# Erikx3/gym_dockauv

Hardware: AMD Instinct MI355X
Metric: env-steps/sec (batched docking3d) (higher is better)
Workload: dtype f32

## Files before the change

gym_dockauv_amd/csrc/dockauv_capi.hip:

```cpp
#include <algorithm>
#include <cmath>
#include <cstdarg>
#include <cstdio>
#include <cstring>

#include "dockauv_capi.h"

using namespace dockauv;

namespace dockauv {

thread_local std::string g_create_error;

int fail(dockauv_handle h, int code, const char* fmt, ...) {
    char buf[512];
    va_list ap;
    va_start(ap, fmt);
    vsnprintf(buf, sizeof buf, fmt, ap);
    va_end(ap);
    if (h) h->err = buf; else g_create_error = buf;
    return code;
}

int check_status(dockauv_handle h) {
    if (!h->status_host) return 0;
    const unsigned int v = *h->status_host;
    if (v != 0)
        return fail(h, DOCKAUV_E_KERNEL, "step kernel status 0x%x: a tail role timed out waiting for its group's integrating wave; "
                    "results since are invalid, destroy the handle", v);
    return 0;
}

int sync_last(dockauv_handle h) {
    if (h->last_stream) HIP_TRY(h, hipStreamSynchronize(h->last_stream)); else HIP_TRY(h, hipDeviceSynchronize());
    return 0;
}

}

namespace {

struct FieldDesc {
    void* base;
    int rows;
    int kind;
};

int dalloc(dockauv_handle h, void** p, size_t bytes) {
    if (bytes == 0) bytes = 256;
    hipError_t e = hipMalloc(p, bytes);
    if (e != hipSuccess) return fail(h, DOCKAUV_E_HIP, "hipMalloc(%zu) failed: %s", bytes, hipGetErrorString(e));
    e = hipMemset(*p, 0, bytes);
    if (e != hipSuccess) return fail(h, DOCKAUV_E_HIP, "hipMemset failed: %s", hipGetErrorString(e));
    h->allocs.push_back(*p);
    return 0;
}

template <typename T>
void fill_vehicle(VehicleP<T>& d, const dockauv_vehicle& v) {
    d.m = (T)v.m;
    d.gWB = (T)(v.W - v.BY);
    d.gx = (T)(v.r_G[0] * v.W - v.r_B[0] * v.BY);
    d.gy = (T)(v.r_G[1] * v.W - v.r_B[1] * v.BY);
    d.gz = (T)(v.r_G[2] * v.W - v.r_B[2] * v.BY);
    for (int i = 0; i < 3; ++i) d.rg[i] = (T)v.r_G[i];
    for (int i = 0; i < 9; ++i) d.Ib[i] = (T)v.I_b[i];
    for (int i = 0; i < 6; ++i) {
        d.ma[i] = (T)v.ma_diag[i];
        d.dl[i] = (T)v.d_lin[i];
        d.dq[i] = (T)v.d_quad[i];
    }
    for (int i = 0; i < 36; ++i) d.Minv[i] = (T)v.M_inv[i];
    for (int i = 0; i < 6 * kMaxU; ++i) d.B[i] = (T)v.B[i];
    for (int i = 0; i < kMaxU; ++i) {
        d.ulo[i] = (T)v.u_lo[i];
        d.uhalf[i] = (T)(v.u_hi[i] - v.u_lo[i]);
    }
    for (int i = 0; i < L_COUNT; ++i) d.lauv[i] = (T)v.lauv[i];
    {
        const double m = v.m, zg = v.r_G[2];
        const double* a = v.ma_diag;
        const double Ix = v.I_b[0], Iy = v.I_b[4], Iz = v.I_b[8];
        const double kc[10] = {m + a[0], m + a[1], m + a[2], m * zg,
                               Iy - Iz + a[4] - a[5], a[1] - a[2],
                               Iz - Ix + a[5] - a[3], a[2] - a[0],
                               Ix - Iy + a[3] - a[4], a[0] - a[1]};
        for (int i = 0; i < 10; ++i) d.kc[i] = (T)kc[i];
    }
    d.n_u = v.n_u;
}

template <typename T>
void fill_env(EnvP<T>& e, const dockauv_env_s& h) {
    const dockauv_config& c = h.cfg;
    e.n_envs = c.n_envs;
    e.max_timesteps = c.max_timesteps;
    e.reward_set = c.reward_set;
    e.reset_mode = c.reset_mode;
    e.scenario = c.scenario;
    e.n_v = c.n_v;
    e.n_h = c.n_h;
    e.blk = c.blocksize_reduce;
    e.n_vr = (c.n_v + c.blocksize_reduce - 1) / c.blocksize_reduce;
    e.n_hr = (c.n_h + c.blocksize_reduce - 1) / c.blocksize_reduce;
    e.n_rays = h.n_rays;
    e.n_red = h.n_red;
    e.n_obs = h.n_obs;
    e.max_cap = c.max_capsules;
    e.max_sph = c.max_spheres;
    e.n_u_max = h.n_u_max;
    e.bf16_wpr = (h.n_obs + 1) / 2 + 2;
    e.bf16_magic = (unsigned)((0x100000000ull / (unsigned)e.bf16_wpr) + 1ull);
    e.seed = c.seed;
    e.h = (T)c.t_step_size;
    e.lp_alpha = (T)(c.t_step_size / (c.t_step_size + c.lowpass_T1));
    e.mu = (T)c.current_mu;
    e.dmax = (T)c.max_dist_from_goal;
    e.dtol = (T)c.dist_goal_reached_tol;
    e.max_att = (T)c.max_attitude;
    e.safety = (T)c.safety_radius;
    for (int i = 0; i < 6; ++i) {
        e.vel_max[i] = (T)c.vel_max[i];
        e.inv_vel[i] = (T)(1.0 / c.vel_max[i]);
    }
    const double eps = 0.001;
    e.inv_dmax = (T)(1.0 / c.max_dist_from_goal);
    e.inv_log_tol = (T)(1.0 / std::log(c.dist_goal_reached_tol / c.max_dist_from_goal));
    e.inv_log_tol_eps = (T)(1.0 / std::log(std::max(c.dist_goal_reached_tol, eps) / c.max_dist_from_goal));
    e.inv_max_att = (T)(1.0 / c.max_attitude);
    e.inv_ray_max = (T)(1.0 / c.radar_max_dist);
    e.w_d = (T)c.w_d;
    e.w_dth = (T)c.w_delta_theta;
    e.w_dpsi = (T)c.w_delta_psi;
    e.w_phi = (T)c.w_phi;
    e.w_th = (T)c.w_theta;
    e.w_thdot = (T)c.w_Thetadot;
    e.w_oa = (T)c.w_oa;
    for (int i = 0; i < 5; ++i) e.w_done[i] = (T)c.w_done[i];
    for (int i = 0; i < kMaxU; ++i) e.w_act[i] = (T)c.action_reward_factors[i];
    e.ray_max = (T)c.radar_max_dist;
    e.alpha_max = (T)c.radar_alpha_max;
    e.beta_max = (T)c.radar_beta_max;
    e.ray_pad_log2 = ceil_log2(h.n_rays);
    e.ray_pad = 1 << e.ray_pad_log2;
    e.device_noise = c.device_noise ? 1 : 0;
    e.fan_cos = (T)h.fan_cos;
    e.fan_sin = (T)h.fan_sin;
    e.sum_beta = (T)h.sum_beta;
}

bool is_symmetric_vehicle(const dockauv_vehicle& v) {
    if (v.r_G[0] != 0.0 || v.r_G[1] != 0.0 || v.r_B[0] != 0.0 || v.r_B[1] != 0.0) return false;
    for (int i = 0; i < 3; ++i)
        for (int j = 0; j < 3; ++j)
            if (i != j && v.I_b[i * 3 + j] != 0.0) return false;
    for (int i = 0; i < 6; ++i)
        for (int j = 0; j < 6; ++j) {
            const bool allowed = (i == j) || (i == 0 && j == 4) || (i == 4 && j == 0) || (i == 1 && j == 3) || (i == 3 && j == 1);
            if (!allowed && std::fabs(v.M_inv[i * 6 + j]) > 1e-14 * std::fabs(v.M_inv[i * 6 + i])) return false;
        }
    return true;
}

bool b_is_diagonal(const dockauv_vehicle& v) {
    if (v.n_u != 6) return false;
    for (int i = 0; i < 6; ++i)
        for (int j = 0; j < kMaxU; ++j)
            if (i != j && v.B[i * kMaxU + j] != 0.0) return false;
    return true;
}

int field_info(dockauv_handle h, int field, FieldDesc* fd, int* width) {
    const dockauv_config& c = h->cfg;
    switch (field) {
        case DOCKAUV_F_STATE: *fd = {h->B.state, 12, 0}; *width = 12; return 0;
        case DOCKAUV_F_U: *fd = {h->B.u, kMaxU, 0}; *width = kMaxU; return 0;
        case DOCKAUV_F_GOAL: *fd = {h->B.goal, 4, 0}; *width = 4; return 0;
        case DOCKAUV_F_CURRENT: *fd = {h->B.cur, 8, 0}; *width = 5; return 0;
        case DOCKAUV_F_TSTEPS: *fd = {h->B.t_steps, 1, 1}; *width = 1; return 0;
        case DOCKAUV_F_CAPSULES: *fd = {h->B.caps, c.max_capsules * 7, 0}; *width = c.max_capsules * 7; return 0;
        case DOCKAUV_F_SPHERES: *fd = {h->B.sph, c.max_spheres * 4, 0}; *width = c.max_spheres * 4; return 0;
        case DOCKAUV_F_VEHICLE_ID: *fd = {h->B.veh_id, 1, 2}; *width = 1; return 0;
        case DOCKAUV_F_CUM_REWARD: *fd = {h->B.cum_reward, 1, 0}; *width = 1; return 0;
        case DOCKAUV_F_EPISODE: *fd = {h->B.episode, 1, 1}; *width = 1; return 0;
        case DOCKAUV_F_CURRENT_SIGMA: *fd = {h->B.cur_sigma, 1, 0}; *width = 1; return 0;
        case DOCKAUV_F_POOL_POSE: *fd = {h->B.p_pose, 6, 0}; *width = 6; return 0;
        case DOCKAUV_F_POOL_GOAL: *fd = {h->B.p_goal, 4, 0}; *width = 4; return 0;
        case DOCKAUV_F_POOL_CURRENT: *fd = {h->B.p_cur, 8, 0}; *width = 5; return 0;
        case DOCKAUV_F_POOL_CAPSULES: *fd = {h->B.p_caps, c.max_capsules * 7, 0}; *width = c.max_capsules * 7; return 0;
        case DOCKAUV_F_POOL_SPHERES: *fd = {h->B.p_sph, c.max_spheres * 4, 0}; *width = c.max_spheres * 4; return 0;
    }
    return fail(h, DOCKAUV_E_INVALID, "unknown field id %d", field);
}

bool is_current_field(int field) { return field == DOCKAUV_F_CURRENT || field == DOCKAUV_F_POOL_CURRENT; }

size_t elem_size(dockauv_handle h, int kind) { return kind == 0 ? h->tsz : (kind == 1 ? 4 : 1); }

void store_elem(dockauv_handle h, int kind, void* dst, size_t idx, double v) {
    if (kind == 0) {
        if (h->f64) static_cast<double*>(dst)[idx] = v; else static_cast<float*>(dst)[idx] = (float)v;
    } else if (kind == 1) {
        static_cast<int32_t*>(dst)[idx] = (int32_t)llround(v);
    } else {
        static_cast<uint8_t*>(dst)[idx] = (uint8_t)llround(v);
    }
}

double load_elem(dockauv_handle h, int kind, const void* src, size_t idx) {
    if (kind == 0) return h->f64 ? static_cast<const double*>(src)[idx] : (double)static_cast<const float*>(src)[idx];
    if (kind == 1) return (double)static_cast<const int32_t*>(src)[idx];
    return (double)static_cast<const uint8_t*>(src)[idx];
}

void set_io(StepIO& d, const dockauv_step_io& s) {
    d.actions = s.actions;
    d.noise = s.noise;
    d.obs = s.obs;
    d.reward = s.reward;
    d.done = s.done;
    d.reward_terms = s.reward_terms;
    d.conditions = s.conditions;
    d.nav = s.nav;
    d.ray_dist = s.ray_dist;
    d.terminal_obs = s.terminal_obs;
    d.state_dot = s.state_dot;
    d.pack = s.pack_reward_done == 2 ? 2 : (s.pack_reward_done ? 1 : 0);
}

int init_handle(dockauv_handle h, const dockauv_config& c, int device) {
    h->cfg = c;
    h->cfg.ray_table = nullptr;
    h->device = device;
    h->f64 = c.precision == DOCKAUV_F64;
    h->tsz = h->f64 ? 8 : 4;
    h->S = ((long)c.n_envs + 63) / 64 * 64;
    h->n_rays = c.n_v * c.n_h;
    {
        double min_bx = 1.0, sb = 0.0;
        for (int r = 0; r < h->n_rays; ++r) {
            const double* q = c.ray_table + (size_t)r * 4;
            const double n = std::sqrt(q[0] * q[0] + q[1] * q[1] + q[2] * q[2]);
            min_bx = std::min(min_bx, q[0] / n);
            sb += q[3];
        }
        const double half = std::min(std::acos(std::max(-1.0, std::min(1.0, min_bx))) + 1e-3, 3.14159265358979);
        h->fan_cos = std::cos(half);
        h->fan_sin = std::sin(half);
        h->sum_beta = sb;
    }
    const int blk = c.blocksize_reduce;
    h->n_red = ((c.n_v + blk - 1) / blk) * ((c.n_h + blk - 1) / blk);
    h->n_obs = DOCKAUV_N_OBS_BASE + h->n_red;
    h->n_u_max = c.vehicle[0].n_u;
    if (c.n_vehicles == 2 && c.vehicle[1].n_u > h->n_u_max) h->n_u_max = c.vehicle[1].n_u;
    h->has_rays = (c.max_capsules + c.max_spheres) > 0;
    h->threads = choose_threads(h->f64, c.n_envs, h->n_rays, c.max_capsules, c.max_spheres, c.n_vehicles, c.threads_per_group);
    if (c.n_vehicles == 2) {
        if (!(c.vehicle[0].kind == DOCKAUV_VEH_CONSTB && b_is_diagonal(c.vehicle[0]) && c.vehicle[1].kind == DOCKAUV_VEH_LAUV))
            return fail(h, DOCKAUV_E_INVALID, "mixed batches support vehicle[0] = diagonal-B (BlueROV2 joystick), vehicle[1] = LAUV");
        h->vk = VK_MIXED;
    } else if (c.vehicle[0].kind == DOCKAUV_VEH_LAUV) {
        h->vk = VK_LAUV;
    } else {
        h->vk = b_is_diagonal(c.vehicle[0]) ? VK_JOY : VK_DENSEB;
    }

    h->sym = true;
    for (int v = 0; v < c.n_vehicles; ++v) h->sym = h->sym && is_symmetric_vehicle(c.vehicle[v]);
    if (c.envs_per_group == -1) h->sym = false;

    const size_t S = (size_t)h->S, t = h->tsz, N = (size_t)c.n_envs;
    const size_t caps = (size_t)c.max_capsules * 7 * S * t, sph = (size_t)c.max_spheres * 4 * S * t;
    Buffers& B = h->B;
    B.stride = h->S;
    void *rays_dev = nullptr, *lt_dev = nullptr, *lc_dev = nullptr, *pdev = nullptr;
    const size_t pbytes = h->f64 ? sizeof(h->a64.P) : sizeof(h->a32.P);
    const size_t stage_bytes[ST_COUNT] = {N * h->n_u_max * t, N * t, N * h->n_obs * 4, N * t, N, N * kNRew * t, N, N * 4 * t,
                                          N * h->n_rays * t, N * h->n_obs * 4, N * 12 * t};
    for (int k = 0; k < ST_COUNT; ++k) h->stage[k].bytes = stage_bytes[k];
    const struct { void** p; size_t bytes; } device_arrays[] = {
        {&B.state, 12 * S * t}, {&B.pos_lo, kLoRows * S * t}, {&B.u, kMaxU * S * t}, {&B.goal, 4 * S * t}, {&B.cur, 8 * S * t},
        {&B.cum_reward, S * t}, {(void**)&B.t_steps, S * 4}, {(void**)&B.episode, S * 4}, {(void**)&B.veh_id, S},
        {&B.cur_sigma, S * t}, {&B.caps, caps}, {&B.sph, sph}, {&B.p_pose, 6 * S * t}, {&B.p_goal, 4 * S * t},
        {&B.p_cur, 8 * S * t}, {&B.p_caps, caps}, {&B.p_sph, sph}, {&rays_dev, (size_t)h->n_rays * 4 * t},
        {&lt_dev, (size_t)64 * 4 * t}, {&lc_dev, (size_t)64 * 4}, {&pdev, pbytes}};
    for (const auto& d : device_arrays)
        if (int rc = dalloc(h, d.p, d.bytes)) return rc;
    for (auto& st : h->stage)
        if (int rc = dalloc(h, &st.dev, st.bytes)) return rc;
    hipError_t e;
    {
        std::vector<unsigned char> tmp((size_t)h->n_rays * 4 * t);
        for (int i = 0; i < h->n_rays * 4; ++i) store_elem(h, 0, tmp.data(), i, c.ray_table[i]);
        e = hipMemcpy(rays_dev, tmp.data(), tmp.size(), hipMemcpyHostToDevice);
        if (e != hipSuccess) return fail(h, DOCKAUV_E_HIP, "ray table upload: %s", hipGetErrorString(e));
    }
    B.rays = rays_dev;
    if (h->n_rays <= 64) {
        const int pad = 1 << ceil_log2(h->n_rays);
        const int n_hr = (c.n_h + blk - 1) / blk;
        std::vector<unsigned char> tmp((size_t)64 * 4 * t);
        int32_t cells[64];
        for (int l = 0; l < 64; ++l) {
            const int r = l % pad;
            const bool ok = r < h->n_rays;
            const double dir[4] = {ok ? c.ray_table[r * 4 + 0] : 1.0, ok ? c.ray_table[r * 4 + 1] : 0.0,
                                   ok ? c.ray_table[r * 4 + 2] : 0.0, ok ? c.ray_table[r * 4 + 3] : 0.0};
            for (int k = 0; k < 4; ++k) store_elem(h, 0, tmp.data(), (size_t)l * 4 + k, dir[k]);
            const int iv = ok ? r / c.n_h : 0, ih = ok ? r % c.n_h : 0;
            cells[l] = (iv / blk) * n_hr + ih / blk;
        }
        e = hipMemcpy(lt_dev, tmp.data(), tmp.size(), hipMemcpyHostToDevice);
        if (e == hipSuccess) e = hipMemcpy(lc_dev, cells, sizeof cells, hipMemcpyHostToDevice);
        if (e != hipSuccess) return fail(h, DOCKAUV_E_HIP, "lane table upload: %s", hipGetErrorString(e));
    }
    B.lane_tab = lt_dev;
    B.lane_cell = static_cast<const int32_t*>(lc_dev);
    {
        void* st_host = nullptr;
        void* st_dev = nullptr;
        e = hipHostMalloc(&st_host, 256, hipHostMallocMapped | hipHostMallocCoherent);
        if (e == hipSuccess) {
            memset(st_host, 0, 256);
            h->pinned_allocs.push_back(st_host);
            e = hipHostGetDevicePointer(&st_dev, st_host, 0);
        }
        if (e != hipSuccess) return fail(h, DOCKAUV_E_HIP, "status word (mapped host memory): %s", hipGetErrorString(e));
        h->status_host = static_cast<volatile unsigned int*>(st_host);
        B.status = static_cast<unsigned int*>(st_dev);
    }
    if (h->f64) {
        fill_env(h->a64.P.E, *h);
        for (int v = 0; v < c.n_vehicles; ++v) {
            fill_vehicle(h->a64.P.V[v], c.vehicle[v]);
            pack_hot(h->a64.P.H[v], h->a64.P.E, h->a64.P.V[v]);
        }
        pack_tail(h->a64.P.Q, h->a64.P.E);
        h->a64.B = B;
    } else {
        fill_env(h->a32.P.E, *h);
        for (int v = 0; v < c.n_vehicles; ++v) {
            fill_vehicle(h->a32.P.V[v], c.vehicle[v]);
            pack_hot(h->a32.P.H[v], h->a32.P.E, h->a32.P.V[v]);
        }
        pack_tail(h->a32.P.Q, h->a32.P.E);
        h->a32.B = B;
    }
    e = hipMemcpy(pdev, h->f64 ? (const void*)&h->a64.P : (const void*)&h->a32.P, pbytes, hipMemcpyHostToDevice);
    if (e != hipSuccess) return fail(h, DOCKAUV_E_HIP, "parameter block upload: %s", hipGetErrorString(e));
    h->a32.params_dev = h->a64.params_dev = pdev;
    const size_t lds = h->f64 ? lds_bytes<double>(64, 512, c.max_capsules, c.max_spheres, h->n_obs, h->has_rays)
                              : lds_bytes<float>(64, 512, c.max_capsules, c.max_spheres, h->n_obs, h->has_rays);
    if (lds > 160 * 1024)
        return fail(h, DOCKAUV_E_INVALID, "configuration needs %zu B of LDS per group (> 160 KiB): fewer rays/obstacles", lds);
    return 0;
}

StepRequest step_request(dockauv_handle h, const dockauv_step_io& io, bool ride) {
    const bool extras = io.noise || io.reward_terms || io.conditions || io.nav || io.ray_dist || io.state_dot || h->trace_dev || h->cfg.device_noise;
    return StepRequest{h->f64, h->sym, h->vk, h->has_rays, h->threads, h->cfg.n_envs, ceil_log2(h->n_rays), h->cfg.reset_mode,
                       h->cfg.reward_set, extras, io.terminal_obs != nullptr, io.pack_reward_done == 2 ? 2 : (io.pack_reward_done ? 1 : 0), ride};
}

}

int dockauv::launch(dockauv_handle h, const dockauv_step_io* io, hipStream_t stream, hipEvent_t ev0, hipEvent_t ev1) {
    int rc;
    StepIO& sio = h->f64 ? h->a64.io : h->a32.io;
    if (h->trace_dev) {
        hipStreamCaptureStatus cap = hipStreamCaptureStatusNone;
        if (hipStreamIsCapturing(stream, &cap) == hipSuccess && cap != hipStreamCaptureStatusNone)
            return fail(h, DOCKAUV_E_INVALID, "the episode-storage trace (dockauv_trace_enable) cannot be recorded into a HIP graph: "
                        "its ring row is a launch argument; disable the trace or launch the steps directly");
    }
    sio.trace = h->trace_dev;
    sio.trace_step = h->trace_dev ? h->trace_step : 0;
    sio.device_noise = (h->cfg.device_noise && !io->noise) ? 1 : 0;
    set_io(sio, *io);
    const StepRequest r = step_request(h, *io, h->a32.ride.plan != nullptr);
    rc = h->f64 ? launch_step_f64(h->a64, r, stream, ev0, ev1) : launch_step_f32(h->a32, r, stream, ev0, ev1);
    if (rc != 0) return fail(h, DOCKAUV_E_HIP, "step kernel launch failed: %s", hipGetErrorString((hipError_t)rc));
    if (h->trace_dev) ++h->trace_step;
    h->last_stream = stream;
    return 0;
}

extern "C" {

int dockauv_abi_version(void) { return DOCKAUV_ABI_VERSION; }

const char* dockauv_build_info(void) {
#define DOCKAUV_STR_(x) #x
#define DOCKAUV_STR(x) DOCKAUV_STR_(x)
    return "libdockauv gfx950 (HIP), abi " DOCKAUV_STR(DOCKAUV_ABI_VERSION) ", built " __DATE__ " " __TIME__;
}

const char* dockauv_last_error(dockauv_handle h) { return h ? h->err.c_str() : g_create_error.c_str(); }

int dockauv_create(const dockauv_config* cfg, int device, dockauv_handle* out) {
    if (!cfg || !out) return fail(nullptr, DOCKAUV_E_INVALID, "null argument");
    *out = nullptr;
    if (cfg->struct_size != sizeof(dockauv_config) || cfg->abi_version != DOCKAUV_ABI_VERSION)
        return fail(nullptr, DOCKAUV_E_INVALID, "dockauv_config size/ABI mismatch: got %u/%u, library has %zu/%d",
                    cfg->struct_size, cfg->abi_version, sizeof(dockauv_config), DOCKAUV_ABI_VERSION);
    const dockauv_config& c = *cfg;
    if (c.n_envs <= 0) return fail(nullptr, DOCKAUV_E_INVALID, "n_envs must be > 0");
    if (c.precision != DOCKAUV_F32 && c.precision != DOCKAUV_F64) return fail(nullptr, DOCKAUV_E_INVALID, "bad precision");
    if (c.n_vehicles < 1 || c.n_vehicles > 2) return fail(nullptr, DOCKAUV_E_INVALID, "n_vehicles must be 1 or 2");
    if (c.max_capsules < 0 || c.max_capsules > DOCKAUV_MAX_CAPSULES) return fail(nullptr, DOCKAUV_E_INVALID, "max_capsules out of range");
    if (c.max_spheres < 0 || c.max_spheres > DOCKAUV_MAX_SPHERES) return fail(nullptr, DOCKAUV_E_INVALID, "max_spheres out of range");
    {
        const uint64_t stride = ((uint64_t)c.n_envs + 63) / 64 * 64;
        uint64_t rows = 12;
        if ((uint64_t)c.max_capsules * 7 > rows) rows = (uint64_t)c.max_capsules * 7;
        if ((uint64_t)c.max_spheres * 4 > rows) rows = (uint64_t)c.max_spheres * 4;
        if (rows * stride * (c.precision == DOCKAUV_F64 ? 8 : 4) >= (1ull << 32))
            return fail(nullptr, DOCKAUV_E_INVALID, "n_envs too large for one handle (an SoA array would exceed 4 GiB): shard the batch over several handles");
    }
    if (c.n_v <= 0 || c.n_h <= 0 || (long)c.n_v * c.n_h > DOCKAUV_MAX_RAYS) return fail(nullptr, DOCKAUV_E_INVALID, "bad ray fan %d x %d", c.n_v, c.n_h);
    if (c.blocksize_reduce <= 0) return fail(nullptr, DOCKAUV_E_INVALID, "blocksize_reduce must be > 0");
    if (c.reward_set != 1 && c.reward_set != 2) return fail(nullptr, DOCKAUV_E_INVALID, "reward_set must be 1 or 2");
    if (c.reset_mode < DOCKAUV_RESET_NONE || c.reset_mode > DOCKAUV_RESET_DEVICE)
        return fail(nullptr, DOCKAUV_E_INVALID, "reset_mode %d not supported by this build", c.reset_mode);
    if (c.scenario < DOCKAUV_SCN_SIMPLE || c.scenario > DOCKAUV_SCN_SPHERES) return fail(nullptr, DOCKAUV_E_INVALID, "bad scenario id %d", c.scenario);
    if (c.reset_mode == DOCKAUV_RESET_DEVICE) {
        static const int need[8] = {0, 0, 1, 1, 5, 4, 5, 0};
        if (c.max_capsules < need[c.scenario]) return fail(nullptr, DOCKAUV_E_INVALID, "scenario %d needs %d capsule slots", c.scenario, need[c.scenario]);
    }
    if (!(c.t_step_size > 0)) return fail(nullptr, DOCKAUV_E_INVALID, "t_step_size must be > 0");
    if (!c.ray_table) return fail(nullptr, DOCKAUV_E_INVALID, "ray_table is NULL");
    for (int v = 0; v < c.n_vehicles; ++v) {
        const dockauv_vehicle& vv = c.vehicle[v];
        if (vv.n_u < 1 || vv.n_u > DOCKAUV_MAX_U) return fail(nullptr, DOCKAUV_E_INVALID, "vehicle %d: n_u out of range", v);
        if (vv.kind != DOCKAUV_VEH_CONSTB && vv.kind != DOCKAUV_VEH_LAUV) return fail(nullptr, DOCKAUV_E_INVALID, "vehicle %d: bad kind", v);
        if (vv.kind == DOCKAUV_VEH_LAUV && vv.n_u != 3) return fail(nullptr, DOCKAUV_E_INVALID, "LAUV needs n_u = 3");
    }

    int ndev = 0;
    hipError_t e = hipGetDeviceCount(&ndev);
    if (e != hipSuccess || ndev <= 0)
        return fail(nullptr, DOCKAUV_E_NODEVICE, "no HIP device available (%s): libdockauv has no CPU fallback",
                    e == hipSuccess ? "count = 0" : hipGetErrorString(e));
    if (device < 0 || device >= ndev) return fail(nullptr, DOCKAUV_E_INVALID, "device %d out of range (have %d)", device, ndev);
    e = hipSetDevice(device);
    if (e != hipSuccess) return fail(nullptr, DOCKAUV_E_HIP, "hipSetDevice: %s", hipGetErrorString(e));

    dockauv_handle h = new dockauv_env_s();
    const int rc = init_handle(h, c, device);
    if (rc != 0) {
        g_create_error = h->err;
        dockauv_destroy(h);
        return rc;
    }
    *out = h;
    return 0;
}

int dockauv_destroy(dockauv_handle h) {
    if (!h) return 0;
    (void)hipSetDevice(h->device);
    (void)hipDeviceSynchronize();
    for (void* p : h->allocs) (void)hipFree(p);
    for (void* p : h->pinned_allocs) (void)hipHostFree(p);
    if (h->host_stream) (void)hipStreamDestroy(h->host_stream);
    if (h->ride_plans_dev) (void)hipFree(h->ride_plans_dev);
    for (void* p : h->trace_allocs) (void)hipFree(p);
    if (h->trace_dev) (void)hipFree(h->trace_dev);
    for (int k = 0; k < 2; ++k) {
        if (h->ev_step[k]) (void)hipEventDestroy(h->ev_step[k]);
        if (h->ev_gather[k]) (void)hipEventDestroy(h->ev_gather[k]);
    }
    delete h;
    return 0;
}

int dockauv_n_obs(dockauv_handle h) { return h ? h->n_obs : DOCKAUV_E_INVALID; }
int dockauv_threads_per_group(dockauv_handle h) { return h ? h->threads : DOCKAUV_E_INVALID; }
int dockauv_n_rays(dockauv_handle h) { return h ? h->n_rays : DOCKAUV_E_INVALID; }
int dockauv_n_u(dockauv_handle h) { return h ? h->n_u_max : DOCKAUV_E_INVALID; }

int dockauv_field_width(dockauv_handle h, int field) {
    if (!h) return DOCKAUV_E_INVALID;
    FieldDesc fd;
    int w = 0;
    int rc = field_info(h, field, &fd, &w);
    return rc ? rc : w;
}

int dockauv_set_field(dockauv_handle h, int field, int first, int count, const double* src) {
    if (!h || !src) return fail(h, DOCKAUV_E_INVALID, "null argument");
    FieldDesc fd;
    int width = 0;
    int rc = field_info(h, field, &fd, &width);
    if (rc) return rc;
    if (first < 0 || count < 0 || (long)first + count > h->cfg.n_envs) return fail(h, DOCKAUV_E_RANGE, "env range [%d, %d) outside [0, %d)", first, first + count, h->cfg.n_envs);
    if (count == 0 || fd.rows == 0) return 0;
    HIP_TRY(h, hipSetDevice(h->device));
    const size_t es = elem_size(h, fd.kind);
    std::vector<unsigned char> tmp((size_t)fd.rows * count * es);
    if (is_current_field(field)) {
        for (int i = 0; i < count; ++i) {
            const double* s = src + (size_t)i * 5;
            const double a = s[3], b = s[4];
            const double row[8] = {s[0], std::cos(a) * std::cos(b), std::sin(b), std::sin(a) * std::cos(b), s[1], s[2], a, b};
            for (int k = 0; k < 8; ++k) store_elem(h, 0, tmp.data(), (size_t)k * count + i, row[k]);
        }
    } else {
        for (int i = 0; i < count; ++i)
            for (int k = 0; k < width; ++k) store_elem(h, fd.kind, tmp.data(), (size_t)k * count + i, src[(size_t)i * width + k]);
    }
    unsigned char* dst = static_cast<unsigned char*>(fd.base) + (size_t)first * es;
    HIP_TRY(h, hipMemcpy2D(dst, (size_t)h->S * es, tmp.data(), (size_t)count * es, (size_t)count * es, fd.rows, hipMemcpyHostToDevice));
    if (field == DOCKAUV_F_STATE) {
        std::vector<unsigned char> lo((size_t)kLoRows * count * es);
        for (int i = 0; i < count; ++i)
            for (int k = 0; k < kLoRows; ++k) {
                const double x = src[(size_t)i * width + kLoState[k]];
                store_elem(h, 0, lo.data(), (size_t)k * count + i, h->f64 ? 0.0 : x - (double)(float)x);
            }
        unsigned char* dlo = static_cast<unsigned char*>(h->B.pos_lo) + (size_t)first * es;
        HIP_TRY(h, hipMemcpy2D(dlo, (size_t)h->S * es, lo.data(), (size_t)count * es, (size_t)count * es, kLoRows, hipMemcpyHostToDevice));
    }
    return 0;
}

int dockauv_get_field(dockauv_handle h, int field, int first, int count, double* dst) {
    if (!h || !dst) return fail(h, DOCKAUV_E_INVALID, "null argument");
    FieldDesc fd;
    int width = 0;
    int rc = field_info(h, field, &fd, &width);
    if (rc) return rc;
    if (first < 0 || count < 0 || (long)first + count > h->cfg.n_envs) return fail(h, DOCKAUV_E_RANGE, "env range [%d, %d) outside [0, %d)", first, first + count, h->cfg.n_envs);
    if (count == 0 || fd.rows == 0) return 0;
    HIP_TRY(h, hipSetDevice(h->device));
    if ((rc = sync_last(h)) != 0 || (rc = check_status(h)) != 0) return rc;
    const size_t es = elem_size(h, fd.kind);
    std::vector<unsigned char> tmp((size_t)fd.rows * count * es);
    const unsigned char* srcp = static_cast<const unsigned char*>(fd.base) + (size_t)first * es;
    HIP_TRY(h, hipMemcpy2D(tmp.data(), (size_t)count * es, srcp, (size_t)h->S * es, (size_t)count * es, fd.rows, hipMemcpyDeviceToHost));
    if (is_current_field(field)) {
        static const int rows[5] = {0, 4, 5, 6, 7};
        for (int i = 0; i < count; ++i)
            for (int k = 0; k < 5; ++k) dst[(size_t)i * 5 + k] = load_elem(h, 0, tmp.data(), (size_t)rows[k] * count + i);
    } else {
        for (int i = 0; i < count; ++i)
            for (int k = 0; k < width; ++k) dst[(size_t)i * width + k] = load_elem(h, fd.kind, tmp.data(), (size_t)k * count + i);
    }
    if (field == DOCKAUV_F_STATE && !h->f64) {
        std::vector<unsigned char> lo((size_t)kLoRows * count * es);
        const unsigned char* slo = static_cast<const unsigned char*>(h->B.pos_lo) + (size_t)first * es;
        HIP_TRY(h, hipMemcpy2D(lo.data(), (size_t)count * es, slo, (size_t)h->S * es, (size_t)count * es, kLoRows, hipMemcpyDeviceToHost));
        for (int i = 0; i < count; ++i)
            for (int k = 0; k < kLoRows; ++k) dst[(size_t)i * width + kLoState[k]] += load_elem(h, 0, lo.data(), (size_t)k * count + i);
    }
    return 0;
}

int dockauv_reset_envs(dockauv_handle h, int first, int count) {
    if (!h) return DOCKAUV_E_INVALID;
    if (first < 0 || count < 0 || (long)first + count > h->cfg.n_envs) return fail(h, DOCKAUV_E_RANGE, "env range outside [0, %d)", h->cfg.n_envs);
    if (count == 0) return 0;
    HIP_TRY(h, hipSetDevice(h->device));
    if (int rc = sync_last(h)) return rc;
    const size_t t = h->tsz, S = (size_t)h->S;
    HIP_TRY(h, hipMemset2D(static_cast<unsigned char*>(h->B.state) + first * t, S * t, 0, count * t, 12));
    HIP_TRY(h, hipMemset2D(static_cast<unsigned char*>(h->B.pos_lo) + first * t, S * t, 0, count * t, kLoRows));
    HIP_TRY(h, hipMemset2D(static_cast<unsigned char*>(h->B.u) + first * t, S * t, 0, count * t, kMaxU));
    HIP_TRY(h, hipMemset(static_cast<unsigned char*>(h->B.cum_reward) + first * t, 0, count * t));
    HIP_TRY(h, hipMemset(h->B.t_steps + first, 0, count * 4));
    std::vector<int32_t> ep(count);
    HIP_TRY(h, hipMemcpy(ep.data(), h->B.episode + first, count * 4, hipMemcpyDeviceToHost));
    for (auto& x : ep) x += 1;
    HIP_TRY(h, hipMemcpy(h->B.episode + first, ep.data(), count * 4, hipMemcpyHostToDevice));
    return 0;
}

int dockauv_step(dockauv_handle h, const dockauv_step_io* io, void* hip_stream) {
    if (!h || !io) return fail(h, DOCKAUV_E_INVALID, "null argument");
    if (!io->actions || !io->obs) return fail(h, DOCKAUV_E_INVALID, "actions/obs must not be NULL");
    if (!io->pack_reward_done && (!io->reward || !io->done)) return fail(h, DOCKAUV_E_INVALID, "reward/done must not be NULL unless pack_reward_done");
    HIP_TRY(h, hipSetDevice(h->device));
    return launch(h, io, (hipStream_t)hip_stream);
}

namespace {
bool sequence_is_resident_material(dockauv_handle h, const dockauv_step_io* ios, int n) {
    if (!h->seq_resident || n < 2) return false;
    for (int i = 0; i < n; ++i) {
        if (select_sequence(step_request(h, ios[i], false)).unsupported || ios[i].reward || ios[i].done) return false;
        if (ios[i].pack_reward_done != ios[0].pack_reward_done) return false;
    }
    return true;
}
}

int dockauv_set_option(dockauv_handle h, int option, int value) {
    if (!h) return DOCKAUV_E_INVALID;
    switch (option) {
        case DOCKAUV_OPT_SEQUENCE_RESIDENT: h->seq_resident = value != 0; return 0;
    }
    return fail(h, DOCKAUV_E_INVALID, "unknown option %d", option);
}

int dockauv_step_sequence(dockauv_handle h, const dockauv_step_io* ios, int n, void* hip_stream) {
    if (!h || !ios || n < 0) return fail(h, DOCKAUV_E_INVALID, "bad argument");
    for (int i = 0; i < n; ++i) {
        if (!ios[i].actions || !ios[i].obs) return fail(h, DOCKAUV_E_INVALID, "step %d: actions/obs must not be NULL", i);
        if (!ios[i].pack_reward_done && (!ios[i].reward || !ios[i].done))
            return fail(h, DOCKAUV_E_INVALID, "step %d: reward/done must not be NULL unless pack_reward_done", i);
    }
    HIP_TRY(h, hipSetDevice(h->device));
    if (sequence_is_resident_material(h, ios, n)) {
        set_io(h->a32.io, ios[0]);
        h->a32.io.trace = nullptr;
        h->a32.io.trace_step = 0;
        h->a32.io.device_noise = 0;
        bool fell_back = false;
        for (int i0 = 0; i0 < n && !fell_back; i0 += kSeqMax) {
            SeqArgs seq;
            seq.n = std::min(kSeqMax, n - i0);
            for (int k = 0; k < kSeqMax; ++k) {
                const int i = i0 + std::min(k, seq.n - 1);
                seq.actions[k] = ios[i].actions;
                seq.obs[k] = ios[i].obs;
            }
            const int rc = launch_sequence_f32(h->a32, step_request(h, ios[0], false), seq, (hipStream_t)hip_stream);
            if (rc == (int)hipErrorNotSupported && i0 == 0) { fell_back = true; break; }
            if (rc != 0) return fail(h, DOCKAUV_E_HIP, "resident step sequence launch failed: %s", hipGetErrorString((hipError_t)rc));
        }
        if (!fell_back) {
            h->last_stream = (hipStream_t)hip_stream;
            return 0;
        }
    }
    for (int i = 0; i < n; ++i) {
        int rc = launch(h, &ios[i], (hipStream_t)hip_stream);
        if (rc) return rc;
    }
    return 0;
}

int dockauv_step_gather_sequence(dockauv_handle h, const dockauv_step_io* ios, int n, const dockauv_p2p_plan* plans,
                                 int n_plans, uint64_t t0, int lag, void* compute_stream, void* gather_stream) {
    if (!h || !ios || !plans || n < 0 || n_plans < 1 || lag < 0 || lag > 1) return fail(h, DOCKAUV_E_INVALID, "bad argument");
    for (int i = 0; i < n; ++i)
        if (!ios[i].actions || !ios[i].obs || !ios[i].pack_reward_done)
            return fail(h, DOCKAUV_E_INVALID, "step %d: actions/obs must not be NULL and pack_reward_done must be set", i);
    {
        const uint64_t row_bytes = (uint64_t)(h->n_obs + 2) * 4u * (uint64_t)h->cfg.n_envs;
        for (int i = 0; i < n; ++i)
            if (ios[i].pack_reward_done != 1)
                return fail(h, DOCKAUV_E_INVALID, "step %d: the peer-to-peer gather ships float32 packed rows (pack_reward_done = 1); "
                            "bfloat16 rows (2) are gathered over RCCL", i);
        for (int k = 0; k < n_plans; ++k)
            if (plans[k].bytes != row_bytes)
                return fail(h, DOCKAUV_E_INVALID, "plan %d: slice of %llu bytes, the handle's packed rows are %llu", k,
                            (unsigned long long)plans[k].bytes, (unsigned long long)row_bytes);
    }
    HIP_TRY(h, hipSetDevice(h->device));
    hipStream_t cs = (hipStream_t)compute_stream, gs = (hipStream_t)gather_stream;
    const bool two = cs != gs;
    if (!two && lag == 1) {
        StepRequest r = step_request(h, dockauv_step_io{}, true);
        if (r.f64 || !r.sym) return fail(h, DOCKAUV_E_INVALID, "lag 1 needs the float kernels of the structural fast path");
        if (needs_full_kernel(r))
            return fail(h, DOCKAUV_E_INVALID, "lag 1 needs the product kernels (no pool reset, reward set 1, fans of 9-16 or 33-64 rays, no logging)");
        for (int i = 0; i < n; ++i) {
            r = step_request(h, ios[i], true);
            if (r.extras || r.terminal_obs)
                return fail(h, DOCKAUV_E_INVALID, "lag 1 needs the product kernels: step %d asks for optional inputs / outputs", i);
        }
        if (n_plans < 4) return fail(h, DOCKAUV_E_INVALID, "lag 1 needs at least 4 plans (gather buffers)");
        for (int i = 1; i < n; ++i)
            if (ios[i].obs == ios[i - 1].obs)
                return fail(h, DOCKAUV_E_INVALID, "step %d: lag 1 needs alternating row buffers (obs of consecutive steps differ)", i);
        for (int k = 0; k < n_plans; ++k)
            if (plans[k].bytes == 0 || plans[k].bytes % 16 != 0 || !plans[k].counter || !plans[k].status || !plans[k].my_flags ||
                plans[k].n_dsts < 1 || plans[k].n_dsts > DOCKAUV_P2P_MAX_PEERS + 1 || plans[k].n_peers < 0 ||
                plans[k].n_peers > DOCKAUV_P2P_MAX_PEERS)
                return fail(h, DOCKAUV_E_INVALID, "plan %d: bad plan (slices must be multiples of 16 bytes)", k);
        const size_t pbytes = sizeof(dockauv_p2p_plan) * (size_t)n_plans;
        if (h->ride_plans_host.size() != pbytes || memcmp(h->ride_plans_host.data(), plans, pbytes) != 0) {
            if (h->ride_plans_host.size() != pbytes) {
                if (h->ride_plans_dev) {
                    HIP_TRY(h, hipStreamSynchronize(cs));
                    HIP_TRY(h, hipFree(h->ride_plans_dev));
                    h->ride_plans_dev = nullptr;
                }
                HIP_TRY(h, hipMalloc(&h->ride_plans_dev, pbytes));
            } else {
                HIP_TRY(h, hipStreamSynchronize(cs));
            }
            HIP_TRY(h, hipMemcpy(h->ride_plans_dev, plans, pbytes, hipMemcpyHostToDevice));
            h->ride_plans_host.assign(reinterpret_cast<const unsigned char*>(plans), reinterpret_cast<const unsigned char*>(plans) + pbytes);
        }
        const unsigned long n16 = plans[0].bytes / 16;
        unsigned long cg = n16 / ((unsigned long)h->threads * 2);
        cg = cg < 8 ? 8 : (cg > 256 ? 256 : cg);
        RideLaunch& ride = h->a32.ride;
        for (int i = 0; i < n; ++i) {
            const uint64_t t = t0 + (uint64_t)i;
            ride = RideLaunch{};
            if (i >= 1) {
                uint32_t stamp = (uint32_t)t;
                if (stamp == 0) stamp = 1;
                ride.plan = static_cast<const dockauv_p2p_plan*>(h->ride_plans_dev) + ((t - 1) % (uint64_t)n_plans);
                ride.src = ios[i - 1].obs;
                ride.stamp = ride.wait_stamp = stamp;
                ride.groups = (int)cg;
            }
            int rc = launch(h, &ios[i], cs);
            ride = RideLaunch{};
            if (rc) return rc;
        }
        if (n >= 1) {
            const uint64_t t = t0 + (uint64_t)(n - 1);
            uint32_t stamp = (uint32_t)(t + 1);
            if (stamp == 0) stamp = 1;
            int rc = launch_gather(&plans[t % (uint64_t)n_plans], ios[n - 1].obs, stamp, stamp, cs);
            if (rc) return fail(h, rc, "%s", g_create_error.c_str());
// ... 254 lines not shown
```

gym_dockauv_amd/csrc/dockauv_device.h:

```cpp
#pragma once
#include <stddef.h>
#include <stdint.h>

namespace dockauv {

constexpr int kMaxU = 8;
constexpr int kNRew = 13;
constexpr int kLoRows = 4;
constexpr int kLoState[kLoRows] = {0, 1, 2, 5};

enum LauvIdx {
    L_Y_r = 0, L_Y_rr, L_Y_urf, L_Z_q, L_Z_qq, L_Z_uqf, L_M_w, L_M_ww, L_M_uw, L_N_v, L_N_vv, L_N_uv,
    L_Y_uv, L_Z_uw, L_M_uqf, L_N_urf, L_Y_uudr, L_Z_uuds, L_M_uuds, L_N_uudr, L_COUNT
};

enum VehKind { VK_JOY = 0, VK_DENSEB = 1, VK_LAUV = 2, VK_MIXED = 3 };

template <typename T>
struct VehicleP {
    T m;
    T gWB, gx, gy, gz;
    T rg[3];
    T Ib[9];
    T ma[6];
    T dl[6], dq[6];
    T Minv[36];
    T B[6 * kMaxU];
    T ulo[kMaxU], uhalf[kMaxU];
    T lauv[L_COUNT];
    T kc[10];
    int n_u;
};

template <typename T>
struct EnvP {
    int n_envs, max_timesteps, reward_set, reset_mode, scenario;
    int n_v, n_h, blk, n_vr, n_hr, n_rays, n_red, n_obs;
    int max_cap, max_sph, n_u_max;
    unsigned long long seed;
    T h, lp_alpha, mu;
    T dmax, dtol, max_att, safety;
    T vel_max[6];
    T inv_dmax, inv_log_tol, inv_log_tol_eps, inv_max_att, inv_ray_max;
    T inv_vel[6];
    T w_d, w_dth, w_dpsi, w_phi, w_th, w_thdot, w_oa;
    T w_done[5];
    T w_act[kMaxU];
    T ray_max, alpha_max, beta_max;
    int bf16_wpr;
    unsigned bf16_magic;
    int ray_pad, ray_pad_log2;
    int device_noise;
    T fan_cos, fan_sin, sum_beta;
};

struct Buffers {
    void* state;
    void* pos_lo;
    void* u;
    void* goal;
    void* cur;
    void* cum_reward;
    int32_t* t_steps;
    int32_t* episode;
    uint8_t* veh_id;
    void* cur_sigma;
    void* caps;
    void* sph;
    void* p_pose;
    void* p_goal;
    void* p_cur;
    void* p_caps;
    void* p_sph;
    const void* rays;
    const void* lane_tab;
    const int32_t* lane_cell;
    unsigned int* status;
    long stride;
};

struct StepIO {
    const void* actions;
    const void* noise;
    float* obs;
    void* reward;
    uint8_t* done;
    void* reward_terms;
    uint8_t* conditions;
    void* nav;
    void* ray_dist;
    float* terminal_obs;
    void* state_dot;
    const void* trace;
    long long trace_step;
    int pack;
    int device_noise;
};

struct TraceDev {
    const int32_t* slot_of_env;
    int n_rows, capacity;
    void* state_pre;
    void* state;
    void* state_dot;
    void* u;
    void* nu_c;
    float* obs;
    void* reward_terms;
    uint8_t* cond;
};

constexpr int minv_sym(int k) {
    const int idx[10] = {0, 4, 7, 9, 14, 19, 21, 24, 28, 35};
    return idx[k];
}
template <typename T>
struct alignas(64) HotP {
    T lp_alpha, mu, h;
    T w_act[kMaxU];
    T ulo[kMaxU], uhalf[kMaxU];
    T bdiag[6];
    T dl[6], dq[6];
    T kc[10];
    T minv[10];
    T gWB, gz;
    T lauv[L_COUNT];
};
static_assert(sizeof(HotP<float>) % 64 == 0 && sizeof(HotP<double>) % 64 == 0, "whole 64-byte lines");

template <typename T>
inline void pack_hot(HotP<T>& H, const EnvP<T>& E, const VehicleP<T>& V) {
    H = HotP<T>{};
    H.lp_alpha = E.lp_alpha; H.mu = E.mu; H.h = E.h;
    for (int i = 0; i < kMaxU; ++i) { H.w_act[i] = E.w_act[i]; H.ulo[i] = V.ulo[i]; H.uhalf[i] = V.uhalf[i]; }
    for (int i = 0; i < 6; ++i) { H.bdiag[i] = V.B[i * kMaxU + i]; H.dl[i] = V.dl[i]; H.dq[i] = V.dq[i]; }
    for (int i = 0; i < 10; ++i) { H.kc[i] = V.kc[i]; H.minv[i] = V.Minv[minv_sym(i)]; }
    H.gWB = V.gWB; H.gz = V.gz;
    for (int i = 0; i < L_COUNT; ++i) H.lauv[i] = V.lauv[i];
}

template <typename T>
struct alignas(64) TailP {
    T inv_log_tol, dtol, dmax, max_att;
    int max_timesteps;
    int reset_mode, n_obs;
    T inv_dmax;
    T ray_max, fan_cos, fan_sin, safety;
    int max_cap, max_sph;
    int ray_pad, ray_pad_log2, n_rays, n_red;
    T inv_ray_max, sum_beta;
    T inv_vel[6], inv_max_att, inv_log_tol_eps;
    T w_d, w_dth, w_dpsi, w_phi, w_th, w_thdot, w_oa;
    T w_done[5];
};
static_assert(sizeof(TailP<float>) == 192 && sizeof(TailP<double>) % 64 == 0, "whole 64-byte lines");

template <typename T>
inline void pack_tail(TailP<T>& Q, const EnvP<T>& E) {
    Q = TailP<T>{};
    Q.inv_dmax = E.inv_dmax; Q.inv_log_tol = E.inv_log_tol; Q.dtol = E.dtol; Q.dmax = E.dmax; Q.max_att = E.max_att;
    Q.max_timesteps = E.max_timesteps; Q.reset_mode = E.reset_mode; Q.n_obs = E.n_obs;
    Q.ray_max = E.ray_max; Q.fan_cos = E.fan_cos; Q.fan_sin = E.fan_sin; Q.safety = E.safety;
    Q.max_cap = E.max_cap; Q.max_sph = E.max_sph;
    Q.ray_pad = E.ray_pad; Q.ray_pad_log2 = E.ray_pad_log2; Q.n_rays = E.n_rays; Q.n_red = E.n_red;
    Q.inv_ray_max = E.inv_ray_max; Q.sum_beta = E.sum_beta;
    for (int i = 0; i < 6; ++i) Q.inv_vel[i] = E.inv_vel[i];
    Q.inv_max_att = E.inv_max_att; Q.inv_log_tol_eps = E.inv_log_tol_eps;
    Q.w_d = E.w_d; Q.w_dth = E.w_dth; Q.w_dpsi = E.w_dpsi; Q.w_phi = E.w_phi; Q.w_th = E.w_th; Q.w_thdot = E.w_thdot;
    Q.w_oa = E.w_oa;
    for (int i = 0; i < 5; ++i) Q.w_done[i] = E.w_done[i];
}

template <typename T, int NV>
struct ParamBlock {
    EnvP<T> E;
    VehicleP<T> V[NV];
    HotP<T> H[NV];
    TailP<T> Q;
};

struct RideLaunch {
    const void* plan = nullptr;
    const void* src = nullptr;
    uint32_t stamp = 0, wait_stamp = 0;
    int groups = 0;
};

constexpr int kSeqMax = 64;
struct SeqArgs {
    const void* actions[kSeqMax];
    float* obs[kSeqMax];
    int n;
};

template <typename T, int NV>
struct KernelArgs {
    ParamBlock<T, NV> P;
    const void* params_dev;
    Buffers B;
    StepIO io;
    RideLaunch ride;
};

struct DevArgs {
    const void* params;
    Buffers B;
    StepIO io;
// ... 365 lines not shown
```

gym_dockauv_amd/csrc/dockauv_step.hip.inc:

```
#include <hip/hip_runtime.h>
#include <hip/hip_ext.h>
#include <math.h>
#include <stdint.h>

#include "dockauv_device.h"
#include "dockauv_ride.h"

namespace dockauv {

__device__ __forceinline__ void sincos_accurate_(float a, float& sn, float& cs) {
    const float j = fmaf(a, 0.636619747f, 12582912.f) - 12582912.f;
    a = fmaf(j, -1.57079601e+00f, a);
    a = fmaf(j, -3.13916473e-07f, a);
    a = fmaf(j, -5.39030253e-15f, a);
    const int i = (int)j;
    const float s = a * a;
    float r = 2.86567956e-6f;
    r = fmaf(r, s, -1.98559923e-4f);
    r = fmaf(r, s, 8.33338592e-3f);
    r = fmaf(r, s, -1.66666672e-1f);
    const float si = fmaf(r, a * s, a);
    float c = 2.44677067e-5f;
    c = fmaf(c, s, -1.38877297e-3f);
    c = fmaf(c, s, 4.16666567e-2f);
    c = fmaf(c, s, -5.00000000e-1f);
    c = fmaf(c, s, 1.0f);
    float so = (i & 1) ? c : si;
    float co = (i & 1) ? si : c;
    sn = (i & 2) ? -so : so;
    cs = ((i + 1) & 2) ? -co : co;
}
__device__ __forceinline__ void sincos_accurate_(double x, double& s, double& c) { sincos(x, &s, &c); }
__device__ __forceinline__ void sincos_(float a, float& sn, float& cs) {
    const float r = a * 0.15915494309189535f;
    sn = __builtin_amdgcn_sinf(r);
    cs = __builtin_amdgcn_cosf(r);
}
__device__ __forceinline__ void sincos_(double x, double& s, double& c) { sincos(x, &s, &c); }
__device__ __forceinline__ float rcp_(float x) { return __builtin_amdgcn_rcpf(x); }
__device__ __forceinline__ double rcp_(double x) { return 1.0 / x; }
__device__ __forceinline__ float div_(float a, float b) { return a * __builtin_amdgcn_rcpf(b); }
__device__ __forceinline__ double div_(double a, double b) { return a / b; }
__device__ __forceinline__ float sqrt_(float x) { return __builtin_amdgcn_sqrtf(x); }
__device__ __forceinline__ double sqrt_(double x) { return sqrt(x); }
__device__ __forceinline__ float rsqrt_(float x) { return __builtin_amdgcn_rsqf(x); }
__device__ __forceinline__ double rsqrt_(double x) { return rcp_(sqrt(x)); }
__device__ __forceinline__ float log_(float x) { return __builtin_amdgcn_logf(x) * 0.6931471805599453f; }
__device__ __forceinline__ double log_(double x) { return log(x); }
__device__ __forceinline__ float atan2_(float y, float x) {
    const float ax = fabsf(x), ay = fabsf(y);
    const float mx = fmaxf(ax, ay), mn = fminf(ax, ay);
    float t = mn * __builtin_amdgcn_rcpf(mx);
    t = (mx == 0.0f) ? 0.0f : t;
    const float s = t * t;
    float p = -0.004054433666169643f;
    p = fmaf(p, s, 0.021862447261810303f);
    p = fmaf(p, s, -0.05591154843568802f);
    p = fmaf(p, s, 0.09642137587070465f);
    p = fmaf(p, s, -0.139086052775383f);
    p = fmaf(p, s, 0.19946560263633728f);
    p = fmaf(p, s, -0.33329859375953674f);
    p = fmaf(p, s, 0.9999993443489075f);
    float a = p * t;
    a = (ay > ax) ? (1.57079632679489662f - a) : a;
    a = (x < 0.0f || (x == 0.0f && __builtin_signbitf(x))) ? (3.14159265358979324f - a) : a;
    return __builtin_copysignf(a, y);
}
__device__ __forceinline__ double atan2_(double y, double x) { return atan2(y, x); }
__device__ __forceinline__ float floor_(float x) { return floorf(x); }
__device__ __forceinline__ double floor_(double x) { return floor(x); }
__device__ __forceinline__ float fma_(float a, float b, float c) { return __builtin_fmaf(a, b, c); }
__device__ __forceinline__ double fma_(double a, double b, double c) { return __builtin_fma(a, b, c); }
__device__ __forceinline__ float abs_(float x) { return fabsf(x); }
__device__ __forceinline__ double abs_(double x) { return fabs(x); }
__device__ __forceinline__ bool isnan_(float x) { return x != x; }
__device__ __forceinline__ bool isnan_(double x) { return x != x; }


template <typename P>
__device__ __forceinline__ __attribute__((address_space(1))) P* uniform_(P* p) {
    const uint64_t v = reinterpret_cast<uint64_t>(p);
    const uint32_t lo = __builtin_amdgcn_readfirstlane((uint32_t)v);
    const uint32_t hi = __builtin_amdgcn_readfirstlane((uint32_t)(v >> 32));
    return (__attribute__((address_space(1))) P*)(((uint64_t)hi << 32) | lo);
}
template <typename P>
__device__ __forceinline__ unsigned row_off_(long k, long S) { return (unsigned)k * (unsigned)S * (unsigned)sizeof(P); }
constexpr int kAfVoff = 1, kAfWriteBack = 2;
template <int AF, typename P>
__device__ __forceinline__ P ldgx_(const P* base, long k, long S, unsigned lane) {
    typedef __attribute__((address_space(1))) const char* gcp;
    constexpr bool VOFF = (AF & kAfVoff) != 0;
    if (VOFF)
        return *reinterpret_cast<__attribute__((address_space(1))) const P*>(
            reinterpret_cast<gcp>(uniform_(reinterpret_cast<const char*>(base))) + (unsigned)(lane * (unsigned)sizeof(P) + row_off_<P>(k, S)));
    return *reinterpret_cast<__attribute__((address_space(1))) const P*>(
        reinterpret_cast<gcp>(uniform_(reinterpret_cast<const char*>(base) + row_off_<P>(k, S))) + lane * (unsigned)sizeof(P));
}
#ifndef DOCKAUV_WT_STORES
#define DOCKAUV_WT_STORES 1
#endif
template <int AF = 0, typename P>
__device__ __forceinline__ void store_global_(__attribute__((address_space(1))) P* p, P v) {
    if (DOCKAUV_WT_STORES && !(AF & kAfWriteBack))
        __hip_atomic_store(p, v, __ATOMIC_RELAXED, __HIP_MEMORY_SCOPE_AGENT);
    else
        *p = v;
}
template <int AF, typename P, typename V>
__device__ __forceinline__ void stgx_(P* base, long k, long S, unsigned lane, V v) {
    typedef __attribute__((address_space(1))) char* gcp;
    constexpr bool VOFF = (AF & kAfVoff) != 0;
    if (VOFF)
        store_global_<AF>(reinterpret_cast<__attribute__((address_space(1))) P*>(
            reinterpret_cast<gcp>(uniform_(reinterpret_cast<char*>(base))) + (unsigned)(lane * (unsigned)sizeof(P) + row_off_<P>(k, S))), (P)v);
    else
        store_global_<AF>(reinterpret_cast<__attribute__((address_space(1))) P*>(
            reinterpret_cast<gcp>(uniform_(reinterpret_cast<char*>(base) + row_off_<P>(k, S))) + lane * (unsigned)sizeof(P)), (P)v);
}
typedef float tile_f32x4 __attribute__((ext_vector_type(4)));
template <int AF = 0>
__device__ __forceinline__ void store_tile16_(float* base, unsigned byte_off, const float4& v) {
    const tile_f32x4 r = {v.x, v.y, v.z, v.w};
    if (DOCKAUV_WT_STORES && !(AF & kAfWriteBack))
        asm volatile("global_store_dwordx4 %0, %1, %2 sc1" ::"v"(byte_off), "v"(r), "s"(base) : "memory");
    else
        asm volatile("global_store_dwordx4 %0, %1, %2" ::"v"(byte_off), "v"(r), "s"(base) : "memory");
}
template <typename P>
__device__ __forceinline__ P ldg_(const P* base, long k, long S, unsigned lane) { return ldgx_<0>(base, k, S, lane); }
template <typename P, typename V>
__device__ __forceinline__ void stg_(P* base, long k, long S, unsigned lane, V v) { stgx_<0>(base, k, S, lane, v); }

template <typename T> __device__ __forceinline__ T pi_() { return T(3.14159265358979323846); }
template <typename T> __device__ __forceinline__ T inf_() { return T(INFINITY); }

template <typename T> __device__ __forceinline__ T clip_(T x, T lo, T hi) { return x < lo ? lo : (x > hi ? hi : x); }
template <typename T> __device__ __forceinline__ T nanmax_(T a, T b) { return (isnan_(a) || a > b) ? a : b; }

template <typename T>
__device__ __forceinline__ T ssa_(T a) {
    const T two_pi = T(2) * pi_<T>();
    T t = a + pi_<T>();
    T k = floor_(t * (T(1) / two_pi));
    T r = t - k * two_pi;
    r = (r < T(0)) ? r + two_pi : r;
    r = (r >= two_pi) ? r - two_pi : r;
    return (a >= -pi_<T>() && a < pi_<T>()) ? a : r - pi_<T>();
}

template <typename T>
struct Trig {
    T sf, cf, st, ct, sp, cp;
};

template <typename T>
__device__ __forceinline__ Trig<T> trig_accurate_(T phi, T th, T psi) {
    Trig<T> g;
    sincos_accurate_(phi, g.sf, g.cf);
    sincos_accurate_(th, g.st, g.ct);
    sincos_accurate_(psi, g.sp, g.cp);
    return g;
}

template <typename T>
__device__ __forceinline__ Trig<T> trig_(T phi, T th, T psi) {
    Trig<T> g;
    sincos_(phi, g.sf, g.cf);
    sincos_(th, g.st, g.ct);
    sincos_(psi, g.sp, g.cp);
    return g;
}

template <typename T>
__device__ __forceinline__ void rotmat_(const Trig<T>& g, T R[9]) {
    R[0] = g.cp * g.ct;
    R[1] = -g.sp * g.cf + g.cp * g.st * g.sf;
    R[2] = g.sp * g.sf + g.cp * g.cf * g.st;
    R[3] = g.sp * g.ct;
    R[4] = g.cp * g.cf + g.sf * g.st * g.sp;
    R[5] = -g.cp * g.sf + g.st * g.sp * g.cf;
    R[6] = -g.st;
    R[7] = g.ct * g.sf;
    R[8] = g.ct * g.cf;
}

template <typename T>
__device__ __forceinline__ void rot_body_to_ned_(const Trig<T>& g, T x, T y, T z, T out[3]) {
    const T y1 = g.cf * y - g.sf * z, z1 = g.sf * y + g.cf * z;
    const T x2 = g.ct * x + g.st * z1, z2 = g.ct * z1 - g.st * x;
    out[0] = g.cp * x2 - g.sp * y1;
    out[1] = g.sp * x2 + g.cp * y1;
    out[2] = z2;
}
template <typename T>
__device__ __forceinline__ void rot_ned_to_body_(const Trig<T>& g, T x, T y, T z, T out[3]) {
    const T x1 = g.cp * x + g.sp * y, y1 = g.cp * y - g.sp * x;
    const T x2 = g.ct * x1 - g.st * z, z2 = g.st * x1 + g.ct * z;
    out[0] = x2;
    out[1] = g.cf * y1 + g.sf * z2;
    out[2] = g.cf * z2 - g.sf * y1;
}

#ifdef DOCKAUV_STAMPS
__device__ unsigned long long g_stamps[64 * 32];
__device__ unsigned long long g_span[16384 * 6];
#define DOCKAUV_SPAN(i)                                                                                    \
    do {                                                                                                   \
        __builtin_amdgcn_sched_barrier(0);                                                                 \
        if ((i) == 2) __builtin_amdgcn_s_waitcnt(0);            \
        if (threadIdx.x == 0 && blockIdx.x < 16384) {                                                      \
            g_span[blockIdx.x * 6 + 2 * (i)] = __builtin_amdgcn_s_memrealtime();                           \
            g_span[blockIdx.x * 6 + 2 * (i) + 1] = __builtin_amdgcn_s_memtime();                           \
        }                                                                                                  \
        __builtin_amdgcn_sched_barrier(0);                                                                 \
    } while (0)
#ifndef DOCKAUV_STAMP_SHIFT
#define DOCKAUV_STAMP_SHIFT 0
#endif
#define DOCKAUV_STAMP_SEL ((blockIdx.x & ((1u << DOCKAUV_STAMP_SHIFT) - 1u)) == 0 && (blockIdx.x >> DOCKAUV_STAMP_SHIFT) < 64)
#define DOCKAUV_STAMP_ROW ((blockIdx.x >> DOCKAUV_STAMP_SHIFT) * 32)
#define DOCKAUV_STAMP(i)                                                                                   \
    do {                                                                                                   \
        __builtin_amdgcn_sched_barrier(0);                                                                 \
        if (threadIdx.x == 0 && DOCKAUV_STAMP_SEL) g_stamps[DOCKAUV_STAMP_ROW + (i)] = __builtin_amdgcn_s_memtime(); \
        __builtin_amdgcn_sched_barrier(0);                                                                 \
    } while (0)
#define DOCKAUV_STAMP_W1(i)                                                                                \
    do {                                                                                                   \
        __builtin_amdgcn_sched_barrier(0);                                                                 \
        if (threadIdx.x == 64 && DOCKAUV_STAMP_SEL) g_stamps[DOCKAUV_STAMP_ROW + (i)] = __builtin_amdgcn_s_memtime(); \
        __builtin_amdgcn_sched_barrier(0);                                                                 \
    } while (0)
#define DOCKAUV_STAMP_WAVES(base)                                                                          \
    do {                                                                                                   \
        __builtin_amdgcn_sched_barrier(0);                                                                 \
        if ((threadIdx.x & 63) == 0 && DOCKAUV_STAMP_SEL) g_stamps[DOCKAUV_STAMP_ROW + (base) + (threadIdx.x >> 6)] = __builtin_amdgcn_s_memtime(); \
        __builtin_amdgcn_sched_barrier(0);                                                                 \
    } while (0)
#define DOCKAUV_STAMP_PIN(i, arr, n)                                        \
    do {                                                                    \
        _Pragma("unroll") for (int k_ = 0; k_ < (n); ++k_) asm volatile("" : "+v"((arr)[k_])); \
        DOCKAUV_STAMP(i);                                                   \
    } while (0)
#else
#define DOCKAUV_SPAN(i) do { } while (0)
#define DOCKAUV_STAMP(i) do { } while (0)
#define DOCKAUV_STAMP_W1(i) do { } while (0)
#define DOCKAUV_STAMP_WAVES(base) do { } while (0)
#define DOCKAUV_STAMP_PIN(i, arr, n) do { } while (0)
#endif

template <typename T, typename VP>
__device__ __forceinline__ void lauv_fin_terms_(const VP& V, const T* u, T tau_c[6]) {
    tau_c[1] = V.lauv[L_Y_uudr] * u[1];
    tau_c[2] = V.lauv[L_Z_uuds] * u[2];
    tau_c[4] = V.lauv[L_M_uuds] * u[2];
    tau_c[5] = V.lauv[L_N_uudr] * u[1];
}
template <typename T, int VK, typename VP>
__device__ __forceinline__ void tau_minus_damping_(const VP& V, const T nu[6], const T tau_c[6], const T* u, T acc[6]) {
    const T u_ = nu[0], v_ = nu[1], w_ = nu[2], p_ = nu[3], q_ = nu[4], r_ = nu[5];
    const T au = abs_(u_), av = abs_(v_), aw = abs_(w_), ap = abs_(p_), aq = abs_(q_), ar = abs_(r_);
    if (VK == VK_LAUV) {
        const auto* L = V.lauv;
        const T uu = u_ * u_;
        acc[0] = u[0] + (V.dl[0] + V.dq[0] * au) * u_;
        acc[1] = tau_c[1] * uu + (V.dl[1] + V.dq[1] * av + L[L_Y_uv] * au) * v_ + (L[L_Y_r] + L[L_Y_rr] * ar + L[L_Y_urf] * au) * r_;
        acc[2] = tau_c[2] * uu + (V.dl[2] + V.dq[2] * aw + L[L_Z_uw] * au) * w_ + (L[L_Z_q] + L[L_Z_qq] * aq + L[L_Z_uqf] * au) * q_;
        acc[3] = (V.dl[3] + V.dq[3] * ap) * p_;
        acc[4] = tau_c[4] * uu + (V.dl[4] + V.dq[4] * aq + L[L_M_uqf] * au) * q_ + (L[L_M_w] + L[L_M_ww] * aw + L[L_M_uw] * au) * w_;
        acc[5] = tau_c[5] * uu + (V.dl[5] + V.dq[5] * ar + L[L_N_urf] * au) * r_ + (L[L_N_v] + L[L_N_vv] * av + L[L_N_uv] * au) * v_;
    } else {
        acc[0] = tau_c[0] + (V.dl[0] + V.dq[0] * au) * u_;
        acc[1] = tau_c[1] + (V.dl[1] + V.dq[1] * av) * v_;
        acc[2] = tau_c[2] + (V.dl[2] + V.dq[2] * aw) * w_;
        acc[3] = tau_c[3] + (V.dl[3] + V.dq[3] * ap) * p_;
        acc[4] = tau_c[4] + (V.dl[4] + V.dq[4] * aq) * q_;
        acc[5] = tau_c[5] + (V.dl[5] + V.dq[5] * ar) * r_;
    }
}

template <typename T, int VK, bool SYM, typename VP>
__device__ __forceinline__ void kinetics_(const VP& V, const T nu[6], const Trig<T>& g, const T tau_c[6],
                                          const T* u, T nud[6]) {
    const T u_ = nu[0], v_ = nu[1], w_ = nu[2], p_ = nu[3], q_ = nu[4], r_ = nu[5];
    T rhs[6];
    tau_minus_damping_<T, VK>(V, nu, tau_c, u, rhs);
    const T ctsf = g.ct * g.sf, ctcf = g.ct * g.cf;
    if (SYM) {
        const auto* K = V.kc;
        const T qw = q_ * w_, rv = r_ * v_, ru = r_ * u_, pw = p_ * w_, pr = p_ * r_, qr = q_ * r_;
        rhs[0] -= K[2] * qw - K[1] * rv + K[3] * pr;
        rhs[1] -= K[0] * ru - K[2] * pw + K[3] * qr;
        rhs[2] -= K[1] * (p_ * v_) - K[0] * (q_ * u_) - K[3] * (p_ * p_ + q_ * q_);
        rhs[3] -= -K[3] * (ru - pw) - K[4] * qr - K[5] * (v_ * w_);
        rhs[4] -= K[3] * (qw - rv) - K[6] * pr - K[7] * (u_ * w_);
        rhs[5] -= -K[8] * (p_ * q_) - K[9] * (u_ * v_);
        rhs[0] -= V.gWB * g.st;
        rhs[1] += V.gWB * ctsf;
        rhs[2] += V.gWB * ctcf;
        rhs[3] -= V.gz * ctsf;
        rhs[4] -= V.gz * g.st;
        nud[0] = V.Minv[0] * rhs[0] + V.Minv[4] * rhs[4];
        nud[1] = V.Minv[7] * rhs[1] + V.Minv[9] * rhs[3];
        nud[2] = V.Minv[14] * rhs[2];
        nud[3] = V.Minv[19] * rhs[1] + V.Minv[21] * rhs[3];
        nud[4] = V.Minv[24] * rhs[0] + V.Minv[28] * rhs[4];
        nud[5] = V.Minv[35] * rhs[5];
    } else {
        const T c1x = q_ * w_ - r_ * v_, c1y = r_ * u_ - p_ * w_, c1z = p_ * v_ - q_ * u_;
        const T t1x = V.rg[1] * r_ - V.rg[2] * q_, t1y = V.rg[2] * p_ - V.rg[0] * r_, t1z = V.rg[0] * q_ - V.rg[1] * p_;
        const T c2x = q_ * t1z - r_ * t1y, c2y = r_ * t1x - p_ * t1z, c2z = p_ * t1y - q_ * t1x;
        const T c3x = V.rg[1] * c1z - V.rg[2] * c1y, c3y = V.rg[2] * c1x - V.rg[0] * c1z, c3z = V.rg[0] * c1y - V.rg[1] * c1x;
        const T ivx = V.Ib[0] * p_ + V.Ib[1] * q_ + V.Ib[2] * r_;
        const T ivy = V.Ib[3] * p_ + V.Ib[4] * q_ + V.Ib[5] * r_;
        const T ivz = V.Ib[6] * p_ + V.Ib[7] * q_ + V.Ib[8] * r_;
        const T c4x = ivy * r_ - ivz * q_, c4y = ivz * p_ - ivx * r_, c4z = ivx * q_ - ivy * p_;
        const T a1x = V.ma[0] * u_, a1y = V.ma[1] * v_, a1z = V.ma[2] * w_;
        const T a2x = V.ma[3] * p_, a2y = V.ma[4] * q_, a2z = V.ma[5] * r_;
        rhs[0] -= V.m * (c1x - c2x) - (a1y * r_ - a1z * q_);
        rhs[1] -= V.m * (c1y - c2y) - (a1z * p_ - a1x * r_);
        rhs[2] -= V.m * (c1z - c2z) - (a1x * q_ - a1y * p_);
        rhs[3] -= V.m * c3x - c4x - (a1y * w_ - a1z * v_) - (a2y * r_ - a2z * q_);
        rhs[4] -= V.m * c3y - c4y - (a1z * u_ - a1x * w_) - (a2z * p_ - a2x * r_);
        rhs[5] -= V.m * c3z - c4z - (a1x * v_ - a1y * u_) - (a2x * q_ - a2y * p_);
        rhs[0] -= V.gWB * g.st;
        rhs[1] += V.gWB * ctsf;
        rhs[2] += V.gWB * ctcf;
        rhs[3] -= -V.gy * ctcf + V.gz * ctsf;
        rhs[4] -= V.gz * g.st + V.gx * ctcf;
        rhs[5] -= -V.gx * ctsf - V.gy * g.st;
#pragma unroll
        for (int i = 0; i < 6; ++i) {
            T acc = T(0);
#pragma unroll
            for (int j = 0; j < 6; ++j) acc += V.Minv[i * 6 + j] * rhs[j];
            nud[i] = acc;
        }
    }
}

template <typename T, int VK, bool SYM, bool WANT_POS, typename VP>
__device__ __forceinline__ void rhs_(const VP& V, const T att[3], const T nu[6], const T nuc[3],
                                     const T tau_c[6], const T* u, T pd[3], T ad[3], T nd[6]) {
    const Trig<T> g = trig_(att[0], att[1], att[2]);
    if (WANT_POS) {
        const T vx = nu[0] + nuc[0], vy = nu[1] + nuc[1], vz = nu[2] + nuc[2];
        rot_body_to_ned_(g, vx, vy, vz, pd);
    }
    const T inv_ct = rcp_(g.ct);
    const T sq_cr = (g.sf * nu[4] + g.cf * nu[5]) * inv_ct;
    ad[0] = nu[3] + sq_cr * g.st;
    ad[1] = g.cf * nu[4] - g.sf * nu[5];
    ad[2] = sq_cr;
    kinetics_<T, VK, SYM>(V, nu, g, tau_c, u, nd);
}
struct NoFetch { __device__ __forceinline__ void operator()() const {} };
template <typename T, int VK, bool SYM, typename VP, typename PIN>
__device__ __forceinline__ void rhs_pinned_(const VP& V, const T att[3], const T nu[6], const T nuc[3], const T tau_c[6],
                                            const T* u, T pd[3], T ad[3], T nd[6], const PIN& before_kinetics) {
    const Trig<T> g = trig_(att[0], att[1], att[2]);
    const T vx = nu[0] + nuc[0], vy = nu[1] + nuc[1], vz = nu[2] + nuc[2];
    rot_body_to_ned_(g, vx, vy, vz, pd);
    const T inv_ct = rcp_(g.ct);
    const T sq_cr = (g.sf * nu[4] + g.cf * nu[5]) * inv_ct;
    ad[0] = nu[3] + sq_cr * g.st;
    ad[1] = g.cf * nu[4] - g.sf * nu[5];
    ad[2] = sq_cr;
    before_kinetics();
    kinetics_<T, VK, SYM>(V, nu, g, tau_c, u, nd);
}

template <typename T, int VK, bool SYM, int VOFF, bool HOTV = false, typename VP, typename EP, typename REQ = NoFetch, typename PIN = NoFetch,
          typename REQT = NoFetch>
__device__ __forceinline__ void vehicle_step_(const VP& V, const EP& E, T y[9], T dpos[3], T u[kMaxU],
                                              const T act[kMaxU], const T nuc[3], T* g_u, long S, unsigned ul, T& psi_lo,
                                              const REQ& request_kinetics = REQ(), const PIN& pin_kinetics = PIN(),
                                              const REQT& request_tail = REQT()) {
    const int n_u = (VK == VK_LAUV) ? 3 : (VK == VK_JOY ? 6 : V.n_u);
    const T one_m_alpha = T(1) - E.lp_alpha;
#pragma unroll
    for (int i = 0; i < kMaxU; ++i) {
        if (i < n_u) {
            const T a = clip_(act[i], T(-1), T(1));
            const T x = V.ulo[i] + V.uhalf[i] * ((a + T(1)) * T(0.5));
            u[i] = E.lp_alpha * x + one_m_alpha * u[i];
            if (!HOTV) stgx_<VOFF>(g_u, i, S, ul, u[i]);
        }
    }
    if (HOTV) {
#pragma unroll
        for (int i = 0; i < kMaxU; ++i)
            if (i < n_u) stgx_<VOFF>(g_u, i, S, ul, u[i]);
    }
    T tau_c[6] = {0, 0, 0, 0, 0, 0};
    if (VK == VK_JOY) {
#pragma unroll
        for (int i = 0; i < 6; ++i) tau_c[i] = V.B[i * kMaxU + i] * u[i];
    } else if (VK == VK_DENSEB) {
#pragma unroll
        for (int i = 0; i < 6; ++i) {
            T acc = T(0);
#pragma unroll
            for (int j = 0; j < kMaxU; ++j)
                if (j < n_u) acc += V.B[i * kMaxU + j] * u[j];
            tau_c[i] = acc;
        }
    } else if (VK == VK_LAUV) {
        lauv_fin_terms_<T>(V, u, tau_c);
    }
    if (HOTV) request_kinetics();
    const T h = E.h;
    const T a21 = h * T(1.0 / 4.0);
    const T a31 = h * T(3.0 / 32.0), a32 = h * T(9.0 / 32.0);
    const T a41 = h * T(1932.0 / 2197.0), a42 = h * T(-7200.0 / 2197.0), a43 = h * T(7296.0 / 2197.0);
    const T a51 = h * T(439.0 / 216.0), a52 = h * T(-8.0), a53 = h * T(3680.0 / 513.0), a54 = h * T(-845.0 / 4104.0);
    const T b1 = h * T(25.0 / 216.0), b3 = h * T(1408.0 / 2565.0), b4 = h * T(2197.0 / 4104.0), b5 = h * T(-1.0 / 5.0);
    T k1[9], k2[9], k3[9], k4[9], pd[3], ys[9];
    DOCKAUV_STAMP_PIN(16, tau_c, 6);
    if (HOTV) rhs_pinned_<T, VK, SYM>(V, y, y + 3, nuc, tau_c, u, pd, k1, k1 + 3, pin_kinetics);
    else rhs_<T, VK, SYM, true>(V, y, y + 3, nuc, tau_c, u, pd, k1, k1 + 3);
    DOCKAUV_STAMP_PIN(17, k1, 9);
#pragma unroll
    for (int i = 0; i < 3; ++i) dpos[i] = b1 * pd[i];
#pragma unroll
    for (int i = 0; i < 9; ++i) ys[i] = y[i] + a21 * k1[i];
    rhs_<T, VK, SYM, false>(V, ys, ys + 3, nuc, tau_c, u, nullptr, k2, k2 + 3);
    DOCKAUV_STAMP_PIN(18, k2, 9);
#pragma unroll
    for (int i = 0; i < 9; ++i) ys[i] = y[i] + a31 * k1[i] + a32 * k2[i];
    rhs_<T, VK, SYM, true>(V, ys, ys + 3, nuc, tau_c, u, pd, k3, k3 + 3);
    DOCKAUV_STAMP_PIN(19, k3, 9);
#pragma unroll
    for (int i = 0; i < 3; ++i) dpos[i] += b3 * pd[i];
#pragma unroll
    for (int i = 0; i < 9; ++i) ys[i] = y[i] + a41 * k1[i] + a42 * k2[i] + a43 * k3[i];
    rhs_<T, VK, SYM, true>(V, ys, ys + 3, nuc, tau_c, u, pd, k4, k4 + 3);
    DOCKAUV_STAMP_PIN(20, k4, 9);
#pragma unroll
    for (int i = 0; i < 3; ++i) dpos[i] += b4 * pd[i];
    constexpr bool PSI2 = sizeof(T) == 4;
    T psi_inc = T(0);
#pragma unroll
    for (int i = 0; i < 9; ++i) {
        ys[i] = y[i] + a51 * k1[i] + a52 * k2[i] + a53 * k3[i] + a54 * k4[i];
        const T inc = b1 * k1[i] + b3 * k3[i] + b4 * k4[i];
        if (PSI2 && i == 2) psi_inc = inc; else y[i] = y[i] + inc;
    }
    rhs_<T, VK, SYM, true>(V, ys, ys + 3, nuc, tau_c, u, pd, k1, k1 + 3);
    DOCKAUV_STAMP_PIN(21, k1, 9);
    if (HOTV) request_tail();
#pragma unroll
    for (int i = 0; i < 3; ++i) dpos[i] += b5 * pd[i];
#pragma unroll
    for (int i = 0; i < 9; ++i)
        if (!(PSI2 && i == 2)) y[i] += b5 * k1[i];
    y[0] = ssa_(y[0]);
    y[1] = ssa_(y[1]);
    if (PSI2) {
        const T b = (psi_inc + b5 * k1[2]) + psi_lo;
        const T s_ = y[2] + b;
        const T bb = s_ - y[2];
        T lo = (y[2] - (s_ - bb)) + (b - bb);
        const T kk = s_ >= pi_<T>() ? T(1) : (s_ < -pi_<T>() ? T(-1) : T(0));
        y[2] = s_ - kk * T(6.2831855f);
        lo -= kk * T(-1.7484555e-7f);
        y[2] = ssa_(y[2]);
        psi_lo = lo;
    } else {
        y[2] = ssa_(y[2]);
    }
}


template <typename T>
struct CapRec {
    T dx, dy, dz, px, py, pz, oa_par, len, r2, oa_top;
};

template <typename T>
__device__ __forceinline__ CapRec<T> load_cap_(const T* cp, int stride) {
    CapRec<T> c;
    c.dx = cp[0 * stride]; c.dy = cp[1 * stride]; c.dz = cp[2 * stride];
    c.px = cp[3 * stride]; c.py = cp[4 * stride]; c.pz = cp[5 * stride];
    c.oa_par = cp[6 * stride]; c.len = cp[7 * stride]; c.r2 = cp[8 * stride]; c.oa_top = cp[9 * stride];
    return c;
}

template <typename T>
__device__ __forceinline__ T ray_capsule_(const CapRec<T>& c, T bx, T by, T bz) {
    const T bard = bx * c.dx + by * c.dy + bz * c.dz;
    const T qx = bx - bard * c.dx, qy = by - bard * c.dy, qz = bz - bard * c.dz;
    const T a = qx * qx + qy * qy + qz * qz;
    const T b = bx * c.px + by * c.py + bz * c.pz;
    const T ra = rcp_(a);
    const T t0 = -b * ra;
    const T ex = c.px + t0 * qx, ey = c.py + t0 * qy, ez = c.pz + t0 * qz;
    const T h = c.r2 - (ex * ex + ey * ey + ez * ez);
    const bool hit = h > T(0);
    const T t = t0 - sqrt_(abs_(h) * ra);
    const T y = c.oa_par + t * bard;
    const bool shaft = (y > T(0)) && (y < c.len);
    T res = t;
    if (__any(hit && !shaft)) {
        const T s = (y >= T(0)) ? c.oa_top : c.oa_par;
        const T ocx = c.px + s * c.dx, ocy = c.py + s * c.dy, ocz = c.pz + s * c.dz;
        const T b2 = bx * ocx + by * ocy + bz * ocz;
        const T fx = ocx - b2 * bx, fy = ocy - b2 * by, fz = ocz - b2 * bz;
        const T h2 = c.r2 - (fx * fx + fy * fy + fz * fz);
        const T cap = (h2 > T(0)) ? (-b2 - sqrt_(abs_(h2))) : T(0);
        res = shaft ? t : cap;
        res = isnan_(y) ? T(-1) : res;
    }
    return (hit && res != T(0)) ? res : -inf_<T>();
}

template <typename T>
__device__ __forceinline__ T ray_sphere_(T ox, T oy, T oz, T r2, T bx, T by, T bz) {
    const T b = ox * bx + oy * by + oz * bz;
    const T ex = ox - b * bx, ey = oy - b * by, ez = oz - b * bz;
    const T hh = r2 - (ex * ex + ey * ey + ez * ez);
    return (hh < T(0)) ? -inf_<T>() : (-b - sqrt_(abs_(hh)));
}

template <int N> struct IntC { static constexpr int value = N; };

__device__ __forceinline__ float wave_sum_to_last_(float x) {
#define DOCKAUV_DPP_ADD(v, ctrl, rmask) ((v) + __builtin_bit_cast(float, __builtin_amdgcn_update_dpp(0, __builtin_bit_cast(int, v), ctrl, rmask, 0xf, false)))
    x = DOCKAUV_DPP_ADD(x, 0x128, 0xf);
    x = DOCKAUV_DPP_ADD(x, 0x124, 0xf);
    x = DOCKAUV_DPP_ADD(x, 0x122, 0xf);
    x = DOCKAUV_DPP_ADD(x, 0x121, 0xf);
    x = DOCKAUV_DPP_ADD(x, 0x142, 0xa);
    x = DOCKAUV_DPP_ADD(x, 0x143, 0xc);
#undef DOCKAUV_DPP_ADD
    return x;
}
__device__ __forceinline__ double wave_sum_to_last_(double x) { return x; }

__device__ __forceinline__ float group_sum_(float x, int width) {
    if (width >= 16) {
#define DOCKAUV_ROW_ROR(v, ctrl) __builtin_bit_cast(float, __builtin_amdgcn_update_dpp(0, __builtin_bit_cast(int, v), ctrl, 0xf, 0xf, false))
        x += DOCKAUV_ROW_ROR(x, 0x128);
        x += DOCKAUV_ROW_ROR(x, 0x124);
        x += DOCKAUV_ROW_ROR(x, 0x122);
        x += DOCKAUV_ROW_ROR(x, 0x121);
#undef DOCKAUV_ROW_ROR
// ... 272 lines not shown
    }
}

template <typename T, int VK, bool SYM, typename VP>
__device__ __forceinline__ void post_step_rhs_(const VP& V, const T st[12], const Trig<T>& g, const T nuc[3], const T* u, T sd[12]) {
    const int n_u = (VK == VK_LAUV) ? 3 : (VK == VK_JOY ? 6 : V.n_u);
    T tau_c[6] = {0, 0, 0, 0, 0, 0};
    if (VK == VK_JOY) {
#pragma unroll
        for (int i = 0; i < 6; ++i) tau_c[i] = V.B[i * kMaxU + i] * u[i];
    } else if (VK == VK_DENSEB) {
#pragma unroll
        for (int i = 0; i < 6; ++i) {
            T acc = T(0);
#pragma unroll
            for (int j = 0; j < kMaxU; ++j)
                if (j < n_u) acc += V.B[i * kMaxU + j] * u[j];
            tau_c[i] = acc;
        }
    } else if (VK == VK_LAUV) {
        lauv_fin_terms_<T>(V, u, tau_c);
    }
    T R[9];
    rotmat_(g, R);
    const T vx = st[6] + nuc[0], vy = st[7] + nuc[1], vz = st[8] + nuc[2];
    sd[0] = R[0] * vx + R[1] * vy + R[2] * vz;
    sd[1] = R[3] * vx + R[4] * vy + R[5] * vz;
    sd[2] = R[6] * vx + R[7] * vy + R[8] * vz;
    const T sq_cr = (g.sf * st[10] + g.cf * st[11]) * rcp_(g.ct);
    sd[3] = st[9] + sq_cr * g.st;
    sd[4] = g.cf * st[10] - g.sf * st[11];
    sd[5] = sq_cr;
    kinetics_<T, VK, SYM>(V, st + 6, g, tau_c, u, sd + 6);
}

template <typename T>
__device__ __forceinline__ T device_normal_(unsigned long long seed, int env, int episode, int t_steps) {
    uint32_t c[4] = {(uint32_t)env, (uint32_t)episode, (uint32_t)t_steps, 1u};
    philox4x32_10_(c, (uint32_t)(seed & 0xffffffffull), (uint32_t)(seed >> 32));
    const T u1 = (T(c[0] >> 8) + T(0.5)) * T(1.0 / 16777216.0);
    const T u2 = T(c[1] >> 8) * T(1.0 / 16777216.0);
    T sn, cs;
    sincos_accurate_(T(2) * pi_<T>() * u2, sn, cs);
    return sqrt_(T(-2) * log_(u1)) * cs;
}

constexpr int kNavSleep = 2;
constexpr int kPrioLevel = 3;
constexpr unsigned kMixedRanks = 0x2310u;
#ifndef DOCKAUV_FAULT_INJECT_DROP_NAV_FLAG
#define DOCKAUV_FAULT_INJECT_DROP_NAV_FLAG 0
#endif

template <typename T, int NT> constexpr int min_waves_() { return sizeof(T) == 4 ? 4 : 1; }

template <int VK, bool RAYS, int EPG, int NT, bool LOG>
constexpr bool early_tail_() {
    return RAYS && (NT / EPG >= 4) && !LOG;
}
template <int VK, bool RAYS, int EPG, int NT, bool LOG>
constexpr bool share_nav_() {
    return early_tail_<VK, RAYS, EPG, NT, LOG>();
}

template <typename T, int VK, bool SYM, bool RAYS, int EPG, int NT, bool LOG, bool TERM, bool WB, int KIND>
constexpr bool hot_params_() {
    if (sizeof(T) != 4 || !SYM || LOG) return false;
    if (VK == VK_LAUV) return !RAYS && NT < 256;
    if (VK != VK_JOY) return false;
    if (KIND == 1) return !(RAYS && NT == 64);
    if (KIND == 2) return RAYS ? NT != 256 : NT == 64;
    return true;
}

template <typename T, int VK, bool SYM, bool RAYS, int EPG, int NT, bool LOG, bool TERM, bool WB, int KIND>
constexpr bool tail_params_() {
    if (!hot_params_<T, VK, SYM, RAYS, EPG, NT, LOG, TERM, WB, KIND>()) return false;
    if (!RAYS || NT / EPG != 4) return false;
    return true;
}

template <typename T, int VK, bool SYM, bool RAYS, int EPG, int NT, bool LOG = false, bool TERM = false, bool WB = false, int KIND = 0>
__device__ __forceinline__ void step_body(const DevArgs& A, const unsigned tix = threadIdx.x, const unsigned bix = blockIdx.x) {
    DOCKAUV_SPAN(0);
    extern __shared__ __align__(16) unsigned char smem_raw[];
    typedef const __attribute__((address_space(4))) ParamBlock<T, 2> CParams;
    CParams* const PB = (CParams*)(uintptr_t)A.params;
    const auto& E = PB->E;
    const Buffers& B = A.B;
    StepIO IO = A.io;
    if (!LOG) {
        IO.noise = nullptr; IO.reward_terms = nullptr; IO.conditions = nullptr; IO.nav = nullptr; IO.ray_dist = nullptr;
        IO.terminal_obs = nullptr; IO.state_dot = nullptr; IO.trace = nullptr; IO.device_noise = 0;
    }
    static_assert(!(TERM && LOG), "the full instantiation writes terminal_obs from its tail roles");
    float* const term_out = TERM ? A.io.terminal_obs : nullptr;
    const long S = B.stride;
    constexpr bool LATE_GOAL = VK == VK_MIXED && !LOG && RAYS;
    constexpr int VOFF = kAfVoff | (WB ? kAfWriteBack : 0);
#ifdef DOCKAUV_STAMPS
    constexpr bool ROTATE = false;
#else
    constexpr bool ROTATE = RAYS && NT / EPG > 1 && NT / EPG < 8;
#endif
    const int tid = ROTATE ? (int)((((tix / EPG) + bix) % (NT / EPG)) * EPG + tix % EPG) : (int)tix;
    const int env0 = bix * EPG;
    const int env = env0 + tid;
    constexpr bool MIXED2 = (VK == VK_MIXED) && (NT / EPG >= 4);
    const bool loader = (MIXED2 ? tid < 2 * EPG : tid < EPG) && (env0 + tid % EPG < A.n_envs);
    bool owner = (tid < EPG) && (env < A.n_envs);
    const int n_valid = min(EPG, A.n_envs - env0);
    const int row_len = E.n_obs + (IO.pack ? 2 : 0);

    DOCKAUV_SPAN(1);
    DOCKAUV_STAMP(0);
#ifdef DOCKAUV_STAMPS
    {
        int probe = A.n_envs;
        asm volatile("" : "+s"(probe));
        DOCKAUV_STAMP(6);
    }
#endif
    constexpr bool SOLO = RAYS && (NT / EPG == 1);
    static_assert(!(SOLO && (LOG || TERM)), "one-wave ray groups exist as plain product kernels only");
    constexpr bool REGREC_OK = SOLO && sizeof(T) == 4;
    const bool regrec = REGREC_OK && solo_regrec(E.max_cap, E.max_sph, E.ray_pad_log2);
    T* lds_pose = reinterpret_cast<T*>(smem_raw);
    T* lds_cap = lds_pose + ((RAYS && !SOLO) ? kPoseFields * EPG : 0);
    T* lds_sph = lds_cap + (RAYS ? kCapFields * E.max_cap * EPG : 0);
    T* lds_oa = lds_sph + (RAYS ? kSphFields * E.max_sph * EPG : 0);
    if (SOLO) {
        size_t rec_bytes = (size_t)(lds_oa - lds_pose) * sizeof(T);
        const size_t tile_bytes = (size_t)EPG * (size_t)(E.n_obs + 2) * sizeof(float);
        rec_bytes = ((rec_bytes > tile_bytes ? rec_bytes : tile_bytes) + 15) & ~(size_t)15;
        lds_oa = reinterpret_cast<T*>(smem_raw + rec_bytes);
    }
    T* lds_col = lds_oa + (RAYS ? (NT / EPG) * 2 * EPG : 0);
    T* lds_act = lds_col + ((RAYS && !SOLO) ? (NT / EPG) * EPG : 0);
    T* lds_hx = lds_act + (RAYS ? (NT / EPG) * EPG : 0);
    T* lds_spec = lds_hx + (NT / EPG >= 2 ? kHxFields * EPG : 0);
    T* lds_nav = lds_oa + 2 * EPG;
    static_assert(!share_nav_<VK, RAYS, EPG, NT, LOG>() || (NT / EPG) * 2 >= 2 + kNavFields, "navigation hand-over needs the spare rows of lds_oa");
    size_t t_bytes = (size_t)(lds_spec + (NT / EPG >= 2 ? kSpecFields * EPG : 0) - lds_pose) * sizeof(T);
    t_bytes = (t_bytes + 15) & ~(size_t)15;
    float* lds_obs = reinterpret_cast<float*>(SOLO ? smem_raw : smem_raw + t_bytes);
    float* const lds_cells = reinterpret_cast<float*>(smem_raw + t_bytes);
    T* const lds_raw = lds_pose;
    auto cell_row = [&](unsigned e, int n_red_) -> float* {
        return (SOLO && !regrec) ? lds_cells + (size_t)e * (unsigned)n_red_ : lds_obs + (size_t)e * row_len + 16;
    };
    T oa_den_r = T(0);

    const unsigned ul = (unsigned)(tid % EPG);
    T* g_state = static_cast<T*>(B.state) + env0;
    T* g_plo = static_cast<T*>(B.pos_lo) + env0;
    T* g_u = static_cast<T*>(B.u) + env0;
    T* g_goal = static_cast<T*>(B.goal) + env0;
    T* g_cur = static_cast<T*>(B.cur) + env0;
    T* g_cum = static_cast<T*>(B.cum_reward) + env0;
    T* g_caps = static_cast<T*>(B.caps) + env0;
    T* g_sph = static_cast<T*>(B.sph) + env0;
    int32_t* g_tsteps = B.t_steps + env0;
    int32_t* g_episode = B.episode + env0;
    constexpr int NU_CT = (VK == VK_LAUV) ? 3 : ((VK == VK_DENSEB) ? 0 : 6);
    const int n_u_max = NU_CT ? NU_CT : E.n_u_max;

    constexpr int W = NT / EPG;
    constexpr bool DUAL = W >= 2;
    constexpr int BK = DUAL ? (W >= 4 ? 3 : 1) : 0;
    constexpr bool QUAD = W >= 4;
    constexpr int OB = QUAD ? (MIXED2 ? 2 : 1) : 0;
    constexpr bool EARLY_ = early_tail_<VK, RAYS, EPG, NT, LOG>();
    constexpr bool FREE_WAVE = EARLY_ && !MIXED2 && W == 4;
    constexpr int RS = QUAD ? (FREE_WAVE ? OB : 2) : BK;
    constexpr bool SHARE_NAV = share_nav_<VK, RAYS, EPG, NT, LOG>();
    const int wv = __builtin_amdgcn_readfirstlane(tid / EPG);
    const unsigned ule = (unsigned)(tid % EPG);
    const bool lane_ok = env0 + (int)ule < A.n_envs;
    const bool bk_lane = (wv == BK) && lane_ok;
    const bool rs_lane = (wv == RS) && lane_ok;
    const bool ob_lane = (wv == OB) && lane_ok;

    T st[12], nuc[3], goal[4];
    T plo[3] = {T(0), T(0), T(0)};
    T psi_lo = T(0);
    T Vc = T(0), edot_norm2 = T(0), act_pen = T(0);
    int t_steps = 0;
    T goal_b[4] = {T(0), T(0), T(0), T(0)}, cum_in = T(0);
    int t_steps_b = 0, episode_in = 0;
    T goal_o[4] = {T(0), T(0), T(0), T(0)};
    int t_steps_o = 0;
    Trig<T> g1{};
    bool collision = false;
    int n_u_env = E.n_u_max;

    T u[kMaxU], act[kMaxU];
    T cdx = T(0), cdy = T(0), cdz = T(0), vmin = T(0), vmax = T(0), w_noise = T(0);
    int vid_l = 0;
    constexpr bool HOT = hot_params_<T, VK, SYM, RAYS, EPG, NT, LOG, TERM, WB, KIND>();
    constexpr bool HOT_WACT = !RAYS;
    HotRegs<T> HR;
    constexpr bool TAIL = tail_params_<T, VK, SYM, RAYS, EPG, NT, LOG, TERM, WB, KIND>();
    constexpr bool NO_PASS = SHARE_NAV && NT / EPG == 4 && !MIXED2;
    constexpr int G0 = kTgDone | kTgAll | (RAYS ? kTgRec : 0) | ((RAYS && !DUAL) ? kTgPass : 0) | (QUAD ? 0 : kTgObs) | (DUAL ? 0 : kTgBk);
    constexpr int GH = kTgAll | (SHARE_NAV ? 0 : kTgDone) | (RAYS ? (kTgRec | kTgPass) : 0) | kTgObs | kTgBk;
    struct {
        T inv_dmax, inv_log_tol, inv_log_tol_eps, inv_max_att, inv_vel[6], dtol, dmax, max_att;
        T w_d, w_dth, w_dpsi, w_phi, w_th, w_thdot, w_oa, w_done[5];
        int max_timesteps, reward_set, n_obs, reset_mode;
    } Q;
    struct {
        int pad, pad_log2, n_rays, n_red, max_cap, max_sph;
        T ray_max, inv_ray_max, sum_beta;
    } RQ;
    if (!TAIL) {
        __builtin_memset(&RQ, 0, sizeof(RQ));
    }
    struct { T ray_max, fan_cos, fan_sin, safety; } RC;
    auto rc_ray_max = [&]() -> T { if constexpr (TAIL) return RC.ray_max; else return E.ray_max; };
    auto rc_fan_cos = [&]() -> T { if constexpr (TAIL) return RC.fan_cos; else return E.fan_cos; };
    auto rc_fan_sin = [&]() -> T { if constexpr (TAIL) return RC.fan_sin; else return E.fan_sin; };
    auto rc_safety = [&]() -> T { if constexpr (TAIL) return RC.safety; else return E.safety; };
    struct { int n_obs, reset_mode; } WQ;
    typedef const __attribute__((address_space(1))) TraceDev GTrace;
    GTrace* const TR = LOG ? (GTrace*)(uintptr_t)IO.trace : nullptr;
    int trace_slot = -1;
    T sigma_l = T(0);
    int episode_l = 0;
    constexpr bool RAISE_PRIO = NT == 256 && RAYS && VK != VK_MIXED && !LOG;
    if (RAISE_PRIO && wv == 0) __builtin_amdgcn_s_setprio(kPrioLevel);
    if (loader) {
        if (VK == VK_MIXED) vid_l = ldgx_<VOFF>(B.veh_id + env0, 0, S, ul);
#pragma unroll
        for (int k = 0; k < 12; ++k)
            if (!(LATE_GOAL && k < 3)) st[k] = ldgx_<VOFF>(g_state, k, S, ul);
        if (sizeof(T) == 4 && !LATE_GOAL) {
#pragma unroll
            for (int k = 0; k < 3; ++k) plo[k] = ldgx_<VOFF>(g_plo, k, S, ul);
        }
        if (sizeof(T) == 4) psi_lo = ldgx_<VOFF>(g_plo, 3, S, ul);
        const T* actp = static_cast<const T*>(IO.actions) + (size_t)env0 * n_u_max;
#pragma unroll
        for (int k = 0; k < kMaxU; ++k) {
            if (k < n_u_max) {
                u[k] = ldgx_<VOFF>(g_u, k, S, ul);
                act[k] = actp[ul * (unsigned)n_u_max + k];
            } else {
                u[k] = T(0);
                act[k] = T(0);
            }
        }
        Vc = ldgx_<VOFF>(g_cur, 0, S, ul);
        cdx = ldgx_<VOFF>(g_cur, 1, S, ul); cdy = ldgx_<VOFF>(g_cur, 2, S, ul); cdz = ldgx_<VOFF>(g_cur, 3, S, ul);
        vmin = ldgx_<VOFF>(g_cur, 4, S, ul); vmax = ldgx_<VOFF>(g_cur, 5, S, ul);
        if (!LATE_GOAL) {
#pragma unroll
            for (int k = 0; k < 4; ++k) goal[k] = ldgx_<VOFF>(g_goal, k, S, ul);
            t_steps = ldgx_<VOFF>(g_tsteps, 0, S, ul);
        }
        w_noise = IO.noise ? ldgx_<VOFF>(static_cast<const T*>(IO.noise) + env0, 0, S, ul) : T(0);
        if (LOG && IO.device_noise) {
            sigma_l = ldgx_<VOFF>(static_cast<const T*>(B.cur_sigma) + env0, 0, S, ul);
            episode_l = ldgx_<VOFF>(g_episode, 0, S, ul);
        }
        if (TR) trace_slot = TR->slot_of_env[env0 + (int)ul];
        DOCKAUV_STAMP(1);
        if constexpr (HOT) fetch_hot_input_<T, VK, HOT_WACT>(PB->H[0], HR);
    }
    if (wv == W - 1) {
        typedef const __attribute__((address_space(4))) unsigned CW;
        CW* const pw = (CW*)(uintptr_t)A.params;
        unsigned param_touch = 0;
        typedef ParamBlock<T, 2> PBlock;
        if (HOT) {
            constexpr int h0 = (int)(__builtin_offsetof(PBlock, H) / 4), hw = (int)(sizeof(HotP<T>) / 4);
#pragma unroll
            for (int off = h0; off < h0 + hw; off += 16) param_touch ^= pw[off];
            if (TAIL) {
                constexpr int q0 = (int)(__builtin_offsetof(PBlock, Q) / 4), qw = (int)(sizeof(TailP<T>) / 4);
#pragma unroll
                for (int off = q0; off < q0 + qw; off += 16) param_touch ^= pw[off];
            }
#pragma unroll
            for (int off = 0; off < (int)(sizeof(EnvP<T>) / 4); off += 16) param_touch ^= pw[off];
        } else {
#pragma unroll
            for (int off = 0; off < (int)(__builtin_offsetof(PBlock, H) / 4); off += 16) param_touch ^= pw[off];
        }
        asm volatile("" ::"s"(param_touch));
    }
    if (bk_lane || rs_lane) {
        if (!SHARE_NAV) {
#pragma unroll
            for (int k = 0; k < 4; ++k) goal_b[k] = ldgx_<VOFF>(g_goal, k, S, ule);
        }
        t_steps_b = ldgx_<VOFF>(g_tsteps, 0, S, ule);
        cum_in = ldgx_<VOFF>(g_cum, 0, S, ule);
        episode_in = ldgx_<VOFF>(g_episode, 0, S, ule);
    }
    if (QUAD && ob_lane && !SHARE_NAV) {
#pragma unroll
        for (int k = 0; k < 4; ++k) goal_o[k] = ldgx_<VOFF>(g_goal, k, S, ule);
        t_steps_o = ldgx_<VOFF>(g_tsteps, 0, S, ule);
    }

    if (RAYS && (!LOG || E.n_rays <= 64)) {
        constexpr int W_ = NT / EPG;
        constexpr int NI = W_ == 1 ? 0 : (MIXED2 ? 2 : 1);
        constexpr int NH = W_ - NI;
        const int hw = wv - NI;
        if ((W_ == 1 && !regrec) || hw >= 0) {
            const int step = W_ == 1 ? 1 : NH, first = W_ == 1 ? 0 : hw;
            const int n_red_z = E.n_red;
            float* orow = cell_row(ule, n_red_z);
            for (int k = first; k < n_red_z; k += step) orow[k] = 0.0f;
            for (int k = first; k < W_ * 2; k += step) lds_oa[k * EPG + ule] = T(0);
            if (first == 0 && !SOLO) {
                lds_pose[14 * EPG + ule] = T(0);
                lds_pose[15 * EPG + ule] = T(0);
                if (SHARE_NAV && ule < 2) lds_nav[4 * EPG + ule] = T(0);
            }
        }
    }
    int ncap_r = 0, nsph_r = 0;
    unsigned cmask_r = 0u, smask_r = 0u;
    T rr[REGREC_OK ? kRegCaps : 1][kCapFields] = {};
    if (RAYS) {
        constexpr int W = NT / EPG;
        const int pw = tid / EPG, pe = tid % EPG;
        const bool pvalid = env0 + pe < A.n_envs;
        if (pvalid && pw == (MIXED2 ? 2 : (W > 1 ? 1 : 0))) {
            int ncap = 0;
            bool open = true;
            for (int c = 0; c < E.max_cap; ++c) {
                const T* cg = g_caps + (size_t)c * 7 * S;
                const unsigned pl = (unsigned)pe;
                const T c1x = ldgx_<VOFF>(cg, 0, S, pl), c1y = ldgx_<VOFF>(cg, 1, S, pl), c1z = ldgx_<VOFF>(cg, 2, S, pl);
                const T bax = ldgx_<VOFF>(cg, 3, S, pl) - c1x, bay = ldgx_<VOFF>(cg, 4, S, pl) - c1y, baz = ldgx_<VOFF>(cg, 5, S, pl) - c1z;
                const T rad = ldgx_<VOFF>(cg, 6, S, pl);
                if (SOLO && regrec) {
                    T* rp = lds_raw + (size_t)c * 7 * EPG + pe;
                    rp[0 * EPG] = c1x; rp[1 * EPG] = c1y; rp[2 * EPG] = c1z;
                    rp[3 * EPG] = bax; rp[4 * EPG] = bay; rp[5 * EPG] = baz;
                    rp[6 * EPG] = rad;
                    open = open && (rad > T(0));
                    ncap = open ? c + 1 : ncap;
                    continue;
                }
                const T len = sqrt_(bax * bax + bay * bay + baz * baz);
                const T inv_len = rcp_(len);
                T* cp = lds_cap + (size_t)c * kCapFields * EPG + pe;
                cp[0 * EPG] = c1x; cp[1 * EPG] = c1y; cp[2 * EPG] = c1z;
                cp[3 * EPG] = bax * inv_len; cp[4 * EPG] = bay * inv_len; cp[5 * EPG] = baz * inv_len;
                cp[6 * EPG] = len;
                cp[7 * EPG] = rad;
                open = open && (rad > T(0));
                ncap = open ? c + 1 : ncap;
            }
            if (SOLO) ncap_r = ncap; else lds_pose[0 * EPG + pe] = T(ncap);
        }
        if (pvalid && pw == (MIXED2 ? 3 : (W > 2 ? 2 : 0))) {
            int nsph = 0;
            bool open = true;
            for (int s_i = 0; s_i < E.max_sph; ++s_i) {
                T rad = T(0);
#pragma unroll
                for (int k = 0; k < 4; ++k) {
                    rad = ldgx_<VOFF>(g_sph, s_i * 4 + k, S, (unsigned)pe);
                    lds_sph[(size_t)(s_i * kSphFields + k) * EPG + pe] = rad;
                }
                open = open && (rad > T(0));
                nsph = open ? s_i + 1 : nsph;
            }
            if (SOLO) nsph_r = nsph; else lds_pose[1 * EPG + pe] = T(nsph);
        }
    }

    if (DUAL && rs_lane && E.reset_mode == 2) {
        T Ub[12], pose_s[6], goal_s[4], cur_s[8], ring_s;
        episode_uniforms_<T>(E, env0 + (int)ule, episode_in + 1, Ub);
        generate_episode_<T>(E, Ub, pose_s, goal_s, cur_s, ring_s);
#pragma unroll
        for (int k = 0; k < 6; ++k) lds_spec[k * EPG + ule] = pose_s[k];
#pragma unroll
        for (int k = 0; k < 4; ++k) lds_spec[(6 + k) * EPG + ule] = goal_s[k];
#pragma unroll
        for (int k = 0; k < 8; ++k) lds_spec[(10 + k) * EPG + ule] = cur_s[k];
        lds_spec[18 * EPG + ule] = ring_s;
    }

    if (MIXED2) owner = loader && (vid_l == wv);
    if (owner) {
        size_t trace_row = 0;
        if (TR && trace_slot >= 0) {
            trace_row = (size_t)(IO.trace_step % TR->capacity) * (size_t)TR->n_rows + (size_t)trace_slot;
            T* sp = static_cast<T*>(TR->state_pre) + trace_row * 12;
#pragma unroll
            for (int k = 0; k < 12; ++k) sp[k] = st[k];
        }
        if (LOG && IO.device_noise && __any(sigma_l != T(0)))
            w_noise = sigma_l * device_normal_<T>(E.seed, env0 + (int)ul, episode_l, t_steps);
        if constexpr (HOT) Vc += (-HR.mu * Vc + w_noise) * HR.h; else Vc += (-E.mu * Vc + w_noise) * E.h;
        Vc = clip_(Vc, vmin, vmax);
        nuc[0] = nuc[1] = nuc[2] = T(0);
        if (__any(Vc != T(0))) {
            const Trig<T> g0 = trig_(st[3], st[4], st[5]);
            rot_ned_to_body_(g0, Vc * cdx, Vc * cdy, Vc * cdz, nuc);
        }
        DOCKAUV_STAMP_PIN(2, nuc, 3);
        T dpos[3];
        int vid = 0;
        if (VK == VK_MIXED) {
            vid = vid_l;
            n_u_env = vid == 0 ? 6 : 3;
        } else {
            n_u_env = (VK == VK_LAUV) ? 3 : (VK == VK_JOY ? 6 : PB->V[0].n_u);
        }
        {
            const T inv_nu = n_u_env == 6 ? T(1.0 / 6.0) : (n_u_env == 3 ? T(1.0 / 3.0) : rcp_(T(n_u_env)));
#pragma unroll
            for (int k = 0; k < kMaxU; ++k) {
                if (k < n_u_env) {
                    const T a = abs_(act[k]) * inv_nu;
                    if constexpr (HOT && HOT_WACT) act_pen += a * a * HR.w_act[k]; else act_pen += a * a * E.w_act[k];
                }
            }
        }
        if constexpr (HOT) {
            vehicle_step_<T, VK, SYM, VOFF, true>(HR.V, HR, st + 3, dpos, u, act, nuc, g_u, S, ul, psi_lo,
                                                  [&]() { request_hot_kinetics_<T, VK>(PB->H[0], HR); },
                                                  [&]() { pin_hot_kinetics_<T, VK>(HR); },
                                                  [&]() { if constexpr (TAIL) request_tail_<G0>(PB->Q, Q, RC, RQ); });
        } else if (VK == VK_MIXED) {
            if (vid == 0) {
                vehicle_step_<T, VK_JOY, SYM, VOFF>(PB->V[0], E, st + 3, dpos, u, act, nuc, g_u, S, ul, psi_lo);
            } else {
                vehicle_step_<T, VK_LAUV, SYM, VOFF>(PB->V[1], E, st + 3, dpos, u, act, nuc, g_u, S, ul, psi_lo);
            }
        } else {
            vehicle_step_<T, VK, SYM, VOFF>(PB->V[0], E, st + 3, dpos, u, act, nuc, g_u, S, ul, psi_lo);
        }
        auto update_position = [&]() {
#pragma unroll
            for (int k = 0; k < 3; ++k) {
                if (sizeof(T) == 4) {
                    const T b = dpos[k] + plo[k];
                    const T s_ = st[k] + b;
                    const T bb = s_ - st[k];
                    plo[k] = (st[k] - (s_ - bb)) + (b - bb);
                    st[k] = s_;
                } else {
                    st[k] += dpos[k];
                }
            }
        };
        if (!LATE_GOAL) update_position();
        DOCKAUV_STAMP_PIN(3, st + 3, 9);
        if (LATE_GOAL) {
#pragma unroll
            for (int k = 0; k < 3; ++k) st[k] = ldgx_<VOFF>(g_state, k, S, ul);
            if (sizeof(T) == 4) {
#pragma unroll
                for (int k = 0; k < 3; ++k) plo[k] = ldgx_<VOFF>(g_plo, k, S, ul);
            }
#pragma unroll
            for (int k = 0; k < 4; ++k) goal[k] = ldgx_<VOFF>(g_goal, k, S, ul);
            t_steps = ldgx_<VOFF>(g_tsteps, 0, S, ul);
        }
        g1 = RAYS ? trig_accurate_(st[3], st[4], st[5]) : trig_(st[3], st[4], st[5]);
        {
            const T sq_cr = (g1.sf * st[10] + g1.cf * st[11]) * rcp_(g1.ct);
            const T e0 = st[9] + sq_cr * g1.st, e1 = g1.cf * st[10] - g1.sf * st[11], e2 = sq_cr;
            edot_norm2 = e0 * e0 + e1 * e1 + e2 * e2;
        }
        if (LATE_GOAL) update_position();
        if (LOG && (IO.state_dot || (TR && trace_slot >= 0))) {
            T uu[kMaxU], sd[12];
#pragma unroll
            for (int k = 0; k < kMaxU; ++k) uu[k] = (k < n_u_env) ? u[k] : T(0);
            if (VK == VK_MIXED) {
                if (vid == 0) post_step_rhs_<T, VK_JOY, SYM>(PB->V[0], st, g1, nuc, uu, sd);
                else post_step_rhs_<T, VK_LAUV, SYM>(PB->V[1], st, g1, nuc, uu, sd);
            } else {
                post_step_rhs_<T, VK, SYM>(PB->V[0], st, g1, nuc, uu, sd);
            }
            if (IO.state_dot) {
                T* o = static_cast<T*>(IO.state_dot) + ((size_t)env0 + ul) * 12;
#pragma unroll
                for (int k = 0; k < 12; ++k) o[k] = sd[k];
            }
            if (TR && trace_slot >= 0) {
                T* o1 = static_cast<T*>(TR->state) + trace_row * 12;
                T* o2 = static_cast<T*>(TR->state_dot) + trace_row * 12;
                T* o3 = static_cast<T*>(TR->u) + trace_row * kMaxU;
                T* o4 = static_cast<T*>(TR->nu_c) + trace_row * 3;
#pragma unroll
                for (int k = 0; k < 12; ++k) { o1[k] = st[k]; o2[k] = sd[k]; }
#pragma unroll
                for (int k = 0; k < kMaxU; ++k) o3[k] = uu[k];
#pragma unroll
                for (int k = 0; k < 3; ++k) o4[k] = nuc[k];
            }
        }
        if constexpr (TAIL) pin_tail_<G0>(Q, RC, RQ);
    }

    if (RAISE_PRIO && wv == 0) __builtin_amdgcn_s_setprio(0);
    if constexpr (TAIL && DUAL) {
        static_assert(NO_PASS, "an integrating wave that takes ray passes would need their scalars here");
        if (wv != 0) {
            request_tail_<GH>(PB->Q, Q, RC, RQ);
            pin_tail_<GH>(Q, RC, RQ);
        }
    }
    if constexpr (TAIL) { WQ.n_obs = PB->Q.n_obs; WQ.reset_mode = PB->Q.reset_mode; }
    constexpr bool LEAN_HX = share_nav_<VK, RAYS, EPG, NT, LOG>();
    auto publish_hx = [&]() {
#pragma unroll
        for (int k = 0; k < 12; ++k)
            if (!(LEAN_HX && (k < 3 || k == 5))) lds_hx[k * EPG + ul] = st[k];
        if (!LEAN_HX) lds_hx[12 * EPG + ul] = Vc;
        lds_hx[13 * EPG + ul] = act_pen;
        lds_hx[14 * EPG + ul] = edot_norm2;
        if (!LEAN_HX) lds_hx[15 * EPG + ul] = collision ? T(1) : T(0);
        if (QUAD) {
#pragma unroll
            for (int k = 0; k < 3; ++k) lds_hx[(16 + k) * EPG + ul] = nuc[k];
            lds_hx[19 * EPG + ul] = g1.sp;
            lds_hx[20 * EPG + ul] = g1.cp;
        }
    };
    if (DUAL && !RAYS) {
        if (owner) publish_hx();
        __builtin_amdgcn_fence(__ATOMIC_RELEASE, "workgroup");
        lds_barrier_<NT>();
    }

    T lr_bx = T(0), lr_by = T(0), lr_bz = T(0), lr_beta = T(0);
    int lr_cell = 0;
    if (RAYS && (!LOG || E.n_rays <= 64)) {
        if (!TAIL) {
            RQ.pad = E.ray_pad; RQ.pad_log2 = E.ray_pad_log2; RQ.n_rays = E.n_rays; RQ.n_red = E.n_red;
            RQ.max_cap = E.max_cap; RQ.max_sph = E.max_sph;
            RQ.ray_max = E.ray_max; RQ.inv_ray_max = E.inv_ray_max; RQ.sum_beta = E.sum_beta;
        }
        if (!(TAIL && NO_PASS && wv == 0)) {
            typedef const __attribute__((address_space(1))) T GT;
            typedef const __attribute__((address_space(1))) int GI;
            GT* const lt = (GT*)(uintptr_t)B.lane_tab + (unsigned)(tid % 64) * 4u;
            lr_bx = lt[0]; lr_by = lt[1]; lr_bz = lt[2]; lr_beta = lt[3];
            lr_cell = ((GI*)(uintptr_t)B.lane_cell)[tid % 64];
        }
    }

    constexpr bool EARLY = EARLY_;
    if constexpr (!TAIL) {
        Q.inv_dmax = E.inv_dmax; Q.inv_log_tol = E.inv_log_tol; Q.inv_log_tol_eps = E.inv_log_tol_eps;
        Q.inv_max_att = E.inv_max_att; Q.dtol = E.dtol; Q.dmax = E.dmax; Q.max_att = E.max_att;
        Q.w_d = E.w_d; Q.w_dth = E.w_dth; Q.w_dpsi = E.w_dpsi; Q.w_phi = E.w_phi; Q.w_th = E.w_th;
        Q.w_thdot = E.w_thdot; Q.w_oa = E.w_oa;
        Q.max_timesteps = E.max_timesteps; Q.reward_set = E.reward_set; Q.n_obs = E.n_obs; Q.reset_mode = E.reset_mode;
#pragma unroll
        for (int k = 0; k < 6; ++k) Q.inv_vel[k] = E.inv_vel[k];
#pragma unroll
        for (int k = 0; k < 5; ++k) Q.w_done[k] = E.w_done[k];
        Q.inv_dmax = pin_sgpr_(Q.inv_dmax); Q.inv_log_tol = pin_sgpr_(Q.inv_log_tol);
        Q.inv_log_tol_eps = pin_sgpr_(Q.inv_log_tol_eps); Q.inv_max_att = pin_sgpr_(Q.inv_max_att);
        Q.dtol = pin_sgpr_(Q.dtol); Q.dmax = pin_sgpr_(Q.dmax); Q.max_att = pin_sgpr_(Q.max_att);
        Q.w_d = pin_sgpr_(Q.w_d); Q.w_dth = pin_sgpr_(Q.w_dth); Q.w_dpsi = pin_sgpr_(Q.w_dpsi);
        Q.w_phi = pin_sgpr_(Q.w_phi); Q.w_th = pin_sgpr_(Q.w_th); Q.w_thdot = pin_sgpr_(Q.w_thdot);
        Q.w_oa = pin_sgpr_(Q.w_oa);
        Q.max_timesteps = pin_sgpr_(Q.max_timesteps); Q.reward_set = pin_sgpr_(Q.reward_set); Q.n_obs = pin_sgpr_(Q.n_obs);
        Q.reset_mode = pin_sgpr_(Q.reset_mode);
#pragma unroll
        for (int k = 0; k < 6; ++k) Q.inv_vel[k] = pin_sgpr_(Q.inv_vel[k]);
#pragma unroll
        for (int k = 0; k < 5; ++k) Q.w_done[k] = pin_sgpr_(Q.w_done[k]);
        WQ.n_obs = Q.n_obs; WQ.reset_mode = Q.reset_mode;
    }

    auto dist2_xy = [](T dx, T dy) { return fma_(dy, dy, dx * dx); };
    auto dist2_xyz = [&](T dx, T dy, T dz) { return fma_(dz, dz, dist2_xy(dx, dy)); };
    auto nav_errors = [&](const T* s_, const T* g_, T& dd, T& dth, T& dpsi) {
        const T dx = g_[0] - s_[0], dy = g_[1] - s_[1], dz = g_[2] - s_[2];
        dd = sqrt_(dist2_xyz(dx, dy, dz));
        const T dxy = sqrt_(dist2_xy(dx, dy));
        dth = s_[4] + atan2_(dz, dxy);
        dpsi = ssa_(atan2_(dy, dx) - s_[5]);
    };
    auto goal_dist = [&](const T* s_, const T* g_) {
        const T dx = g_[0] - s_[0], dy = g_[1] - s_[1], dz = g_[2] - s_[2];
        return sqrt_(dist2_xyz(dx, dy, dz));
    };
    auto conditions = [&](T dd, const T* s_, int tsteps, bool col) -> int {
        const bool c0 = dd < Q.dtol;
        const bool c1 = dd > Q.dmax;
        const bool c2 = (abs_(s_[3]) > Q.max_att) || (abs_(s_[4]) > Q.max_att);
        const bool c3 = tsteps >= Q.max_timesteps;
        return (c0 ? 1 : 0) | (c1 ? 2 : 0) | (c2 ? 4 : 0) | (c3 ? 8 : 0) | (col ? 16 : 0);
    };

    auto trace_obs_row = [&](unsigned lane) -> float* {
        if (!TR) return nullptr;
        const int slot = TR->slot_of_env[env0 + (int)lane];
        if (slot < 0) return nullptr;
        return TR->obs + ((size_t)(IO.trace_step % TR->capacity) * (size_t)TR->n_rows + (size_t)slot) * (size_t)Q.n_obs;
    };
    int* const nav_flags = reinterpret_cast<int*>(lds_nav + 4 * EPG);
    auto raise_nav_flag_ = [&](int which) {
        if (DOCKAUV_FAULT_INJECT_DROP_NAV_FLAG && bix == 0) return;
        __builtin_amdgcn_fence(__ATOMIC_RELEASE, "workgroup", "local");
        __hip_atomic_store(reinterpret_cast<int*>(lds_nav + 4 * EPG + which), 1, __ATOMIC_RELAXED, __HIP_MEMORY_SCOPE_WORKGROUP);
    };
    auto wait_nav_ = [&]() {
        unsigned spins = 0;
        for (;;) {
            int f = __hip_atomic_load(nav_flags, __ATOMIC_RELAXED, __HIP_MEMORY_SCOPE_WORKGROUP);
            if (MIXED2) f &= __hip_atomic_load(reinterpret_cast<int*>(lds_nav + 4 * EPG + 1), __ATOMIC_RELAXED, __HIP_MEMORY_SCOPE_WORKGROUP);
            if (__builtin_amdgcn_readfirstlane(f) != 0) break;
            if (++spins > (1u << 18)) {
                const int me = (int)__builtin_amdgcn_mbcnt_hi(~0u, __builtin_amdgcn_mbcnt_lo(~0u, 0u));
                if (me == __builtin_amdgcn_readfirstlane(me))
                    __hip_atomic_fetch_or(B.status, 1u, __ATOMIC_RELAXED, __HIP_MEMORY_SCOPE_SYSTEM);
                break;
            }
            __builtin_amdgcn_s_sleep(kNavSleep);
        }
        __builtin_amdgcn_fence(__ATOMIC_ACQUIRE, "workgroup", "local");
    };
    auto wait_nav = wait_nav_;
    bool ob_zero_row = false;
    auto obs_ray_cells = [&](bool zero_row, unsigned lane) {
        if (TERM) return;
        float* ot = lds_obs + (size_t)lane * row_len;
        if (SOLO && regrec) {
            if (zero_row)
                for (int k = 16; k < Q.n_obs; ++k) ot[k] = 0.0f;
            return;
        }
        if (SOLO) {
            const float* cr = lds_cells + (size_t)lane * (unsigned)(Q.n_obs - 16);
            for (int k = 16; k < Q.n_obs; ++k) ot[k] = zero_row ? 0.0f : cr[k - 16];
            return;
        }
        if (zero_row && IO.terminal_obs) {
            float* to = IO.terminal_obs + (size_t)env0 * Q.n_obs + lane * (unsigned)Q.n_obs;
            for (int k = 16; k < Q.n_obs; ++k) to[k] = ot[k];
        }
        if (float* tro = trace_obs_row(lane))
            for (int k = 16; k < Q.n_obs; ++k) tro[k] = ot[k];
        if (zero_row)
            for (int k = 16; k < Q.n_obs; ++k) ot[k] = 0.0f;
    };
    auto obs_rest = [&](const T* s_, const T* nuc_, T sp_, T cp_, bool zero_row, unsigned lane, bool lazy_done = false) {
        float* ot = lds_obs + (size_t)lane * row_len;
        T o[16];
        o[3] = clip_(s_[6] * Q.inv_vel[0], T(-1), T(1));
        o[4] = clip_(s_[7] * Q.inv_vel[1], T(-1), T(1));
        o[5] = clip_(s_[8] * Q.inv_vel[2], T(-1), T(1));
        o[6] = clip_(s_[3] * Q.inv_max_att, T(-1), T(1));
        o[7] = clip_(s_[4] * Q.inv_max_att, T(-1), T(1));
        o[8] = clip_(sp_, T(-1), T(1));
        o[9] = clip_(cp_, T(-1), T(1));
        o[10] = clip_(s_[9] * Q.inv_vel[3], T(-1), T(1));
        o[11] = clip_(s_[10] * Q.inv_vel[4], T(-1), T(1));
        o[12] = clip_(s_[11] * Q.inv_vel[5], T(-1), T(1));
        o[13] = clip_(nuc_[0] * T(0.5), T(-1), T(1));
        o[14] = clip_(nuc_[1] * T(0.5), T(-1), T(1));
        o[15] = clip_(nuc_[2] * T(0.5), T(-1), T(1));
        if (SHARE_NAV && lazy_done && !TERM) {
#pragma unroll
            for (int k = 3; k < 16; ++k) asm volatile("" : "+v"(o[k]));
            wait_nav_();
            zero_row = (lds_nav[3 * EPG + lane] != T(0)) && Q.reset_mode != 0;
            ob_zero_row = zero_row;
        }
        if (TERM) zero_row = false;
        if (zero_row && IO.terminal_obs) {
            float* to = IO.terminal_obs + (size_t)env0 * Q.n_obs + lane * (unsigned)Q.n_obs;
#pragma unroll
            for (int k = 3; k < 16; ++k) to[k] = (float)o[k];
            if (!RAYS)
                for (int k = 16; k < Q.n_obs; ++k) to[k] = 1.0f;
        }
        if (float* tro = trace_obs_row(lane)) {
#pragma unroll
            for (int k = 3; k < 16; ++k) tro[k] = (float)o[k];
            if (!RAYS)
                for (int k = 16; k < Q.n_obs; ++k) tro[k] = 1.0f;
        }
#pragma unroll
        for (int k = 3; k < 16; ++k) ot[k] = zero_row ? 0.0f : (float)o[k];
        if (!RAYS) {
            const float fill = zero_row ? 0.0f : 1.0f;
            int k = 16;
            if ((row_len & 1) == 0)
                for (; k + 2 <= Q.n_obs; k += 2) *reinterpret_cast<float2*>(ot + k) = make_float2(fill, fill);
            for (; k < Q.n_obs; ++k) ot[k] = fill;
            if (IO.ray_dist)
                for (int r = 0; r < E.n_rays; ++r) (static_cast<T*>(IO.ray_dist) + (size_t)env0 * E.n_rays)[lane * (unsigned)E.n_rays + r] = E.ray_max;
        }
    };

    auto col_from_records = [&](unsigned lane) -> bool {
        bool c = false;
#pragma unroll
        for (int w = 0; w < W; ++w) c = c || (lds_col[w * EPG + lane] != T(0));
        return c;
    };

    auto w0_tail = [&]() {
        DOCKAUV_STAMP(4);
        T dd, dth, dpsi;
        nav_errors(st, goal, dd, dth, dpsi);
        float* ot = lds_obs + (size_t)ul * row_len;
        const T o0 = clip_(T(1) - log_(dd * Q.inv_dmax) * Q.inv_log_tol, T(0), T(1));
        const T o1 = clip_(dth * (T(2) / pi_<T>()), T(-1), T(1));
        const T o2 = clip_(dpsi * (T(1) / pi_<T>()), T(-1), T(1));
        const int cbits0 = conditions(dd, st, t_steps, collision);
        const bool done = cbits0 != 0;
        const bool zero_row = done && Q.reset_mode != 0;
        if (SHARE_NAV) {
            lds_nav[0 * EPG + ul] = dd;
            lds_nav[1 * EPG + ul] = dth;
            lds_nav[2 * EPG + ul] = dpsi;
            lds_nav[3 * EPG + ul] = T(cbits0);
            raise_nav_flag_(MIXED2 ? wv : 0);
        }
        if (zero_row && IO.terminal_obs) {
            float* to = IO.terminal_obs + (size_t)env0 * Q.n_obs + ul * (unsigned)Q.n_obs;
            to[0] = (float)o0; to[1] = (float)o1; to[2] = (float)o2;
        }
        if (float* tro = trace_obs_row(ul)) {
            tro[0] = (float)o0; tro[1] = (float)o1; tro[2] = (float)o2;
        }
        const bool zero_tile = zero_row && !TERM;
        ot[0] = zero_tile ? 0.0f : (float)o0;
        ot[1] = zero_tile ? 0.0f : (float)o1;
        ot[2] = zero_tile ? 0.0f : (float)o2;
        if (!QUAD) {
            obs_rest(st, nuc, g1.sp, g1.cp, zero_row, ul);
            if (RAYS) obs_ray_cells(zero_row, ul);
        }
        if (DUAL && !zero_row) {
#pragma unroll
            for (int k = 0; k < 12; ++k) stgx_<VOFF>(g_state, k, S, ul, st[k]);
            stgx_<VOFF>(g_cur, 0, S, ul, Vc);
        }
        if (sizeof(T) == 4) {
#pragma unroll
            for (int k = 0; k < 3; ++k) stgx_<VOFF>(g_plo, k, S, ul, zero_row ? T(0) : plo[k]);
            stgx_<VOFF>(g_plo, 3, S, ul, zero_row ? T(0) : psi_lo);
        }
        DOCKAUV_STAMP(5);
    };

    auto ob_tail_pre = [&]() {
        if (QUAD && ob_lane) {
            T so[12], nuco[3];
#pragma unroll
            for (int k = 0; k < 12; ++k) so[k] = lds_hx[k * EPG + ule];
#pragma unroll
            for (int k = 0; k < 3; ++k) nuco[k] = lds_hx[(16 + k) * EPG + ule];
            if (SHARE_NAV) {
                obs_rest(so, nuco, lds_hx[19 * EPG + ule], lds_hx[20 * EPG + ule], false, ule, true);
            } else {
                const bool col = EARLY ? col_from_records(ule) : (lds_hx[15 * EPG + ule] != T(0));
                const bool done = conditions(goal_dist(so, goal_o), so, t_steps_o, col) != 0;
                ob_zero_row = done && Q.reset_mode != 0;
                obs_rest(so, nuco, lds_hx[19 * EPG + ule], lds_hx[20 * EPG + ule], ob_zero_row, ule);
            }
        }
    };
    auto ob_tail_post = [&]() {
        if (QUAD && RAYS && ob_lane) obs_ray_cells(ob_zero_row, ule);
    };

    T bk_rw[kNRew], bk_part = T(0);
    int bk_cbits = 0;
    auto role_inputs = [&](T* sb, T& Vc_b, T& act_pen_b, T& edot_b, bool& col_b) {
        if (DUAL) {
#pragma unroll
            for (int k = 0; k < 12; ++k) sb[k] = lds_hx[k * EPG + ule];
            Vc_b = lds_hx[12 * EPG + ule];
            act_pen_b = lds_hx[13 * EPG + ule];
            edot_b = lds_hx[14 * EPG + ule];
            col_b = EARLY ? col_from_records(ule) : (lds_hx[15 * EPG + ule] != T(0));
        } else {
#pragma unroll
            for (int k = 0; k < 12; ++k) sb[k] = st[k];
            Vc_b = Vc; act_pen_b = act_pen; edot_b = edot_norm2; col_b = collision;
        }
    };
    T bk_dd = T(0), bk_dth = T(0), bk_dpsi = T(0), bk_psi = T(0);
    auto bk_tail_pre = [&]() {
        if (!bk_lane) return;
        T sb[12], Vc_b, act_pen_b, edot_b;
        bool col_b;
        role_inputs(sb, Vc_b, act_pen_b, edot_b, col_b);
        T* rw = bk_rw;
        {
            const T a = sb[3] * (T(2) / pi_<T>()), b = sb[4] * (T(2) / pi_<T>());
            rw[3] = -Q.w_phi * (a * a);
            rw[4] = -Q.w_th * (b * b);
            const T e = sqrt_(edot_b) * Q.inv_vel[3];
            rw[5] = -Q.w_thdot * (e * e);
        }
        rw[6] = T(0);
        rw[7] = -act_pen_b;
        T dd, dth, dpsi;
        int cbits;
        if (SHARE_NAV) {
            wait_nav();
            dd = lds_nav[0 * EPG + ule]; dth = lds_nav[1 * EPG + ule]; dpsi = lds_nav[2 * EPG + ule];
            cbits = (int)lds_nav[3 * EPG + ule];
        } else {
            nav_errors(sb, goal_b, dd, dth, dpsi);
            cbits = conditions(dd, sb, t_steps_b, col_b);
        }
        bk_dd = dd; bk_dth = dth; bk_dpsi = dpsi; bk_psi = sb[5];
        bk_cbits = cbits;
        const T eps = T(0.001);
        const T log_dd_e = log_((dd > eps ? dd : eps) * Q.inv_dmax);
        const T lp_d = T(1) - clip_(log_dd_e * Q.inv_log_tol_eps, T(0), T(1));
        bk_part = lp_d;
        rw[0] = -Q.w_d * lp_d;
        const T half_pi = pi_<T>() / T(2);
        if (LOG && Q.reward_set == 2) {
            const T ath = abs_(dth), aps = abs_(dpsi);
            const T l_th = T(1) - clip_(div_(log_((ath > eps ? ath : eps) / half_pi), log_(eps / half_pi)), T(0), T(1));
            const T l_ps = T(1) - clip_(div_(log_((aps > eps ? aps : eps) / pi_<T>()), log_(eps / pi_<T>())), T(0), T(1));
            const T ld2 = lp_d * lp_d, ld4 = ld2 * ld2;
            const T t2 = l_th * l_th, p2 = l_ps * l_ps;
            rw[1] = -Q.w_dth * (t2 * t2) * ld4;
            rw[2] = -Q.w_dpsi * (p2 * p2) * ld4;
        } else {
            const T a = dth * (T(2) / pi_<T>()), b = dpsi * (T(1) / pi_<T>());
            rw[1] = -Q.w_dth * (a * a);
            rw[2] = -Q.w_dpsi * (b * b);
        }
#pragma unroll
        for (int k = 0; k < 5; ++k) rw[8 + k] = (cbits >> k & 1) ? Q.w_done[k] : T(0);
    };
    auto bk_tail_post = [&]() {
        if (!bk_lane) return;
        T* rw = bk_rw;
        const int cbits = bk_cbits;
        const bool done = cbits != 0;
        const bool reset_now = done && Q.reset_mode != 0;
        T oa = T(0);
        if (RAYS) {
            T sum_beta = T(0), denom = T(0);
#pragma unroll
            for (int w = 0; w < (LOG ? NT / EPG : 1); ++w) {
                if (REGREC_OK && regrec) {
                    sum_beta += E.sum_beta;
                    denom += oa_den_r;
                    continue;
                }
                sum_beta += lds_oa[(w * 2 + 0) * EPG + ule];
                denom += lds_oa[(w * 2 + 1) * EPG + ule];
            }
            oa = div_(sum_beta, denom) - T(1);
        }
        if (LOG && Q.reward_set == 2) {
            const T eps = T(0.001);
            const T aoa = abs_(oa);
            const T l_oa = T(1) - clip_(div_(log_(aoa > eps ? aoa : eps), log_(eps)), T(0), T(1));
            const T ld2 = bk_part * bk_part, ld4 = ld2 * ld2;
            const T o2 = l_oa * l_oa;
            rw[6] = -Q.w_oa * (o2 * o2) * ld4;
        } else {
            rw[6] = -Q.w_oa * oa;
        }
        T reward = T(0);
#pragma unroll
        for (int k = 0; k < kNRew; ++k) reward += rw[k];

        if (!RAYS && DUAL) DOCKAUV_STAMP_W1(11);
        if (IO.reward) stgx_<VOFF>(static_cast<T*>(IO.reward) + env0, 0, S, ule, reward);
        if (IO.done) stgx_<VOFF>(IO.done + env0, 0, S, ule, (uint8_t)(done ? 1 : 0));
        if (IO.pack) {
            float* ot = lds_obs + (size_t)ule * row_len;
            ot[Q.n_obs] = (float)reward;
            ot[Q.n_obs + 1] = done ? 1.0f : 0.0f;
        }
        if (IO.conditions) stgx_<VOFF>(IO.conditions + env0, 0, S, ule, (uint8_t)cbits);
        if (IO.reward_terms) {
            T* rt = static_cast<T*>(IO.reward_terms) + (size_t)env0 * kNRew + ule * (unsigned)kNRew;
#pragma unroll
            for (int k = 0; k < kNRew; ++k) rt[k] = rw[k];
        }
        if (TR) {
            const int slot = TR->slot_of_env[env0 + (int)ule];
            if (slot >= 0) {
                const size_t row = (size_t)(IO.trace_step % TR->capacity) * (size_t)TR->n_rows + (size_t)slot;
                T* rt = static_cast<T*>(TR->reward_terms) + row * kNRew;
#pragma unroll
                for (int k = 0; k < kNRew; ++k) rt[k] = rw[k];
                TR->cond[row] = (uint8_t)cbits;
            }
        }
        if (IO.nav) {
            T* nv = static_cast<T*>(IO.nav) + (size_t)env0 * 4 + ule * 4u;
            nv[0] = bk_dd; nv[1] = bk_dth; nv[2] = bk_dpsi; nv[3] = ssa_(goal_b[3] - bk_psi);
        }
        stgx_<VOFF>(g_cum, 0, S, ule, reset_now ? T(0) : cum_in + reward);
        stgx_<VOFF>(g_tsteps, 0, S, ule, reset_now ? 0 : t_steps_b + 1);
    };
    auto rs_tail = [&]() {
        if (!rs_lane) return;
        DOCKAUV_STAMP(7);
        T sb[12], Vc_b, act_pen_b, edot_b;
        bool col_b;
        role_inputs(sb, Vc_b, act_pen_b, edot_b, col_b);
        bool done;
        if (SHARE_NAV) {
            wait_nav();
            done = lds_nav[3 * EPG + ule] != T(0);
        } else {
            done = (QUAD ? conditions(goal_dist(sb, goal_b), sb, t_steps_b, col_b) : bk_cbits) != 0;
        }
        const bool reset_now = done && Q.reset_mode != 0;
        if (reset_now) {
            const int ep_next = episode_in + 1;
            T curv[8];
            if (LOG && Q.reset_mode == 1) {
                const T* pp = static_cast<const T*>(B.p_pose);
                const T* pg = static_cast<const T*>(B.p_goal);
                const T* pc = static_cast<const T*>(B.p_cur);
#pragma unroll
                for (int k = 0; k < 6; ++k) sb[k] = ldgx_<VOFF>(pp + env0, k, S, ule);
#pragma unroll
                for (int k = 0; k < 4; ++k) goal_b[k] = ldgx_<VOFF>(pg + env0, k, S, ule);
#pragma unroll
                for (int k = 0; k < 8; ++k) curv[k] = ldgx_<VOFF>(pc + env0, k, S, ule);
                const T* pcap = static_cast<const T*>(B.p_caps);
                for (int k = 0; k < E.max_cap * 7; ++k) stgx_<VOFF>(g_caps, (size_t)k, S, ule, ldgx_<VOFF>(pcap + env0, (size_t)k, S, ule));
                const T* psp = static_cast<const T*>(B.p_sph);
                for (int k = 0; k < E.max_sph * 4; ++k) stgx_<VOFF>(g_sph, (size_t)k, S, ule, ldgx_<VOFF>(psp + env0, (size_t)k, S, ule));
            } else {
                T ring_s;
                if (DUAL) {
#pragma unroll
                    for (int k = 0; k < 6; ++k) sb[k] = lds_spec[k * EPG + ule];
#pragma unroll
                    for (int k = 0; k < 4; ++k) goal_b[k] = lds_spec[(6 + k) * EPG + ule];
#pragma unroll
                    for (int k = 0; k < 8; ++k) curv[k] = lds_spec[(10 + k) * EPG + ule];
                    ring_s = lds_spec[18 * EPG + ule];
                } else {
                    T Ub[12];
                    episode_uniforms_<T>(E, env0 + (int)ule, ep_next, Ub);
                    generate_episode_<T>(E, Ub, sb, goal_b, curv, ring_s);
                }
                store_capsules_<T>(E, g_caps, S, ule, ring_s);
            }
#pragma unroll
            for (int k = 6; k < 12; ++k) sb[k] = T(0);
#pragma unroll
            for (int k = 0; k < kMaxU; ++k)
                if (k < n_u_max) stgx_<VOFF>(g_u, k, S, ule, T(0));
#pragma unroll
            for (int k = 0; k < 4; ++k) stgx_<VOFF>(g_goal, k, S, ule, goal_b[k]);
#pragma unroll
            for (int k = 1; k < 8; ++k) stgx_<VOFF>(g_cur, k, S, ule, curv[k]);
            Vc_b = curv[0];
            stgx_<VOFF>(g_episode, 0, S, ule, ep_next);
        }
        if (!DUAL || reset_now) {
#pragma unroll
            for (int k = 0; k < 12; ++k) stgx_<VOFF>(g_state, k, S, ule, sb[k]);
            stgx_<VOFF>(g_cur, 0, S, ule, Vc_b);
        }
    };

    if (RAYS) {
        DOCKAUV_STAMP(14);
        if (owner && !SOLO) {
            T R1[9];
            rotmat_(g1, R1);
            lds_pose[2 * EPG + ul] = st[0];
            lds_pose[3 * EPG + ul] = st[1];
            lds_pose[4 * EPG + ul] = st[2];
#pragma unroll
            for (int k = 0; k < 9; ++k) lds_pose[(5 + k) * EPG + ul] = R1[k];
        }
        if (!SOLO) lds_barrier_<NT>();
        if constexpr (TAIL) { WQ.n_obs = pin_sgpr_(WQ.n_obs); WQ.reset_mode = pin_sgpr_(WQ.reset_mode); }
        if (env0 + (int)ule < A.n_envs) {
            const T* P = lds_pose + ule;
            const int ncap = SOLO ? ncap_r : (int)P[0 * EPG], nsph = SOLO ? nsph_r : (int)P[1 * EPG];
            const T px0 = SOLO ? st[0] : P[2 * EPG], py0 = SOLO ? st[1] : P[3 * EPG], pz0 = SOLO ? st[2] : P[4 * EPG];
            T R1[9];
            if (SOLO) {
                rotmat_(g1, R1);
            } else {
#pragma unroll
                for (int k = 0; k < 9; ++k) R1[k] = P[(5 + k) * EPG];
            }
            bool col = false;
            auto complete_capsule = [&](T c1x, T c1y, T c1z, T dx, T dy, T dz, T len, T rad, T* o, bool& hits_body) -> bool {
                const T oax = px0 - c1x, oay = py0 - c1y, oaz = pz0 - c1z;
                const T oa_par = oax * dx + oay * dy + oaz * dz;
                const T px = oax - oa_par * dx, py = oay - oa_par * dy, pz = oaz - oa_par * dz;
                o[0] = R1[0] * dx + R1[3] * dy + R1[6] * dz;
                o[1] = R1[1] * dx + R1[4] * dy + R1[7] * dz;
                o[2] = R1[2] * dx + R1[5] * dy + R1[8] * dz;
                o[3] = R1[0] * px + R1[3] * py + R1[6] * pz;
                o[4] = R1[1] * px + R1[4] * py + R1[7] * pz;
                o[5] = R1[2] * px + R1[5] * py + R1[8] * pz;
                o[6] = oa_par;
                o[7] = len;
                o[8] = rad * rad;
                o[9] = oa_par - len;
                const bool may = capsule_may_be_hit_<T>(o[0], o[3], px * px + py * py + pz * pz, oa_par, len, rad, rc_ray_max(),
                                                        rc_fan_cos(), rc_fan_sin());
                const T s_ = -oa_par, t_ = oa_par - len;
                T hh = s_ > t_ ? s_ : t_;
                hh = hh > T(0) ? hh : T(0);
                const T dist = sqrt_(hh * hh + (px * px + py * py + pz * pz));
                hits_body = dist <= rad + rc_safety();
                return may;
            };
            if (REGREC_OK && regrec) {
#pragma unroll
                for (int c = 0; c < kRegCaps; ++c) {
                    if (c < E.max_cap) {
                        const T* rp = lds_raw + (size_t)c * 7 * EPG + ule;
                        const T bax = rp[3 * EPG], bay = rp[4 * EPG], baz = rp[5 * EPG];
                        const T len = sqrt_(bax * bax + bay * bay + baz * baz);
                        const T inv_len = rcp_(len);
                        bool hb;
                        const bool may = complete_capsule(rp[0 * EPG], rp[1 * EPG], rp[2 * EPG], bax * inv_len, bay * inv_len, baz * inv_len,
                                                          len, rp[6 * EPG], rr[c], hb);
                        if (c < ncap && may) cmask_r |= 1u << c;
                        col = col || (c < ncap && hb);
                    }
                }
            }
            for (int c = wv; c < ((REGREC_OK && regrec) ? 0 : ncap); c += W) {
                T* cp = lds_cap + (size_t)c * kCapFields * EPG + ule;
                const T c1x = cp[0 * EPG], c1y = cp[1 * EPG], c1z = cp[2 * EPG];
                const T dx = cp[3 * EPG], dy = cp[4 * EPG], dz = cp[5 * EPG];
                const T len = cp[6 * EPG], rad = cp[7 * EPG];
                const T oax = px0 - c1x, oay = py0 - c1y, oaz = pz0 - c1z;
                const T oa_par = oax * dx + oay * dy + oaz * dz;
                const T px = oax - oa_par * dx, py = oay - oa_par * dy, pz = oaz - oa_par * dz;
                cp[0 * EPG] = R1[0] * dx + R1[3] * dy + R1[6] * dz;
                cp[1 * EPG] = R1[1] * dx + R1[4] * dy + R1[7] * dz;
                cp[2 * EPG] = R1[2] * dx + R1[5] * dy + R1[8] * dz;
                cp[3 * EPG] = R1[0] * px + R1[3] * py + R1[6] * pz;
                cp[4 * EPG] = R1[1] * px + R1[4] * py + R1[7] * pz;
                cp[5 * EPG] = R1[2] * px + R1[5] * py + R1[8] * pz;
                cp[6 * EPG] = oa_par;
                cp[7 * EPG] = len;
                cp[8 * EPG] = rad * rad;
                cp[9 * EPG] = oa_par - len;
                if (capsule_may_be_hit_<T>(cp[0 * EPG], cp[3 * EPG], px * px + py * py + pz * pz, oa_par, len, rad, rc_ray_max(),
                                           rc_fan_cos(), rc_fan_sin())) {
                    if (SOLO) cmask_r |= 1u << c;
                    else atomicOr(reinterpret_cast<unsigned int*>(lds_pose + 14 * EPG + ule), 1u << c);
                }
                const T s_ = -oa_par, t_ = oa_par - len;
                T hh = s_ > t_ ? s_ : t_;
                hh = hh > T(0) ? hh : T(0);
                const T dist = sqrt_(hh * hh + (px * px + py * py + pz * pz));
                col = col || (dist <= rad + rc_safety());
            }
            for (int s_i = wv; s_i < nsph; s_i += W) {
                T* sp = lds_sph + (size_t)s_i * kSphFields * EPG + ule;
                const T cx = sp[0 * EPG], cy = sp[1 * EPG], cz = sp[2 * EPG], rad = sp[3 * EPG];
                const T ocx = px0 - cx, ocy = py0 - cy, ocz = pz0 - cz;
                const T d2 = ocx * ocx + ocy * ocy + ocz * ocz;
                sp[0 * EPG] = R1[0] * ocx + R1[3] * ocy + R1[6] * ocz;
                sp[1 * EPG] = R1[1] * ocx + R1[4] * ocy + R1[7] * ocz;
                sp[2 * EPG] = R1[2] * ocx + R1[5] * ocy + R1[8] * ocz;
                sp[3 * EPG] = rad * rad;
                const T dist = sqrt_(d2);
                if (sphere_may_be_hit_<T>(sp[0 * EPG], d2, dist, rad, rc_ray_max(), rc_fan_cos(), rc_fan_sin())) {
                    if (SOLO) smask_r |= 1u << s_i;
                    else atomicOr(reinterpret_cast<unsigned int*>(lds_pose + 15 * EPG + ule), 1u << s_i);
                }
                col = col || (dist <= rc_safety() + rad);
            }
            if (SOLO) collision = col; else lds_col[wv * EPG + ule] = col ? T(1) : T(0);
            DOCKAUV_STAMP(15);
        }
        if (REGREC_OK && regrec) {
            const int n_red_z = E.n_red;
            float* orow = cell_row(ule, n_red_z);
            for (int k = 0; k < n_red_z; ++k) orow[k] = 0.0f;
        }
        if (EARLY && owner) {
            publish_hx();
            __builtin_amdgcn_fence(__ATOMIC_RELEASE, "workgroup");
        }
    }

    if (RAYS) {
        lds_barrier_<NT>();
        if (owner) {
            if (!SOLO) {
#pragma unroll
                for (int w = 0; w < W; ++w) collision = collision || (lds_col[w * EPG + ul] != T(0));
            }
            if (DUAL && !EARLY) {
                publish_hx();
                __builtin_amdgcn_fence(__ATOMIC_RELEASE, "workgroup");
            }
            if (EARLY) w0_tail();
        }
        if (SHARE_NAV && MIXED2 && wv < 2) raise_nav_flag_(wv);
        typedef const __attribute__((address_space(4))) T CT;
        CT* const rays = (CT*)(uintptr_t)B.rays;
        DOCKAUV_STAMP_W1(10);
        static_assert(EPG % 64 == 0, "a wave must not straddle two ray indices");
        if (SHARE_NAV && NT / EPG == 4 && !MIXED2 && wv == 0) {
        } else if (!LOG || E.n_rays <= 64) {
            const int pad = pin_sgpr_(RQ.pad), pad_log2 = pin_sgpr_(RQ.pad_log2), n_rays = pin_sgpr_(RQ.n_rays);
            const int n_red = pin_sgpr_(RQ.n_red), max_cap = pin_sgpr_(RQ.max_cap), max_sph = pin_sgpr_(RQ.max_sph);
            const T ray_max = pin_sgpr_(RQ.ray_max), inv_ray_max = pin_sgpr_(RQ.inv_ray_max), sum_beta_all = pin_sgpr_(RQ.sum_beta);
            const int lane = tid % 64;
            const int r = lane & (pad - 1), sub = lane >> pad_log2;
            const bool ray_ok = r < n_rays;
            const T bx = lr_bx, by = lr_by, bz = lr_bz, beta = lr_beta;
// ... 588 lines not shown
```

Measured before the change: 7.599 billion.

## Interleave per-env state rows in pairs and quads for vectorized global access

```diff
diff --git a/gym_dockauv_amd/csrc/dockauv_capi.hip b/gym_dockauv_amd/csrc/dockauv_capi.hip
--- a/gym_dockauv_amd/csrc/dockauv_capi.hip
+++ b/gym_dockauv_amd/csrc/dockauv_capi.hip
@@ -44,6 +44,7 @@
     void* base;
     int rows;
     int kind;
+    int vec;
 };
 
 int dalloc(dockauv_handle h, void** p, size_t bytes) {
@@ -173,22 +174,22 @@
 int field_info(dockauv_handle h, int field, FieldDesc* fd, int* width) {
     const dockauv_config& c = h->cfg;
     switch (field) {
-        case DOCKAUV_F_STATE: *fd = {h->B.state, 12, 0}; *width = 12; return 0;
-        case DOCKAUV_F_U: *fd = {h->B.u, kMaxU, 0}; *width = kMaxU; return 0;
-        case DOCKAUV_F_GOAL: *fd = {h->B.goal, 4, 0}; *width = 4; return 0;
-        case DOCKAUV_F_CURRENT: *fd = {h->B.cur, 8, 0}; *width = 5; return 0;
-        case DOCKAUV_F_TSTEPS: *fd = {h->B.t_steps, 1, 1}; *width = 1; return 0;
-        case DOCKAUV_F_CAPSULES: *fd = {h->B.caps, c.max_capsules * 7, 0}; *width = c.max_capsules * 7; return 0;
-        case DOCKAUV_F_SPHERES: *fd = {h->B.sph, c.max_spheres * 4, 0}; *width = c.max_spheres * 4; return 0;
-        case DOCKAUV_F_VEHICLE_ID: *fd = {h->B.veh_id, 1, 2}; *width = 1; return 0;
-        case DOCKAUV_F_CUM_REWARD: *fd = {h->B.cum_reward, 1, 0}; *width = 1; return 0;
-        case DOCKAUV_F_EPISODE: *fd = {h->B.episode, 1, 1}; *width = 1; return 0;
-        case DOCKAUV_F_CURRENT_SIGMA: *fd = {h->B.cur_sigma, 1, 0}; *width = 1; return 0;
-        case DOCKAUV_F_POOL_POSE: *fd = {h->B.p_pose, 6, 0}; *width = 6; return 0;
-        case DOCKAUV_F_POOL_GOAL: *fd = {h->B.p_goal, 4, 0}; *width = 4; return 0;
-        case DOCKAUV_F_POOL_CURRENT: *fd = {h->B.p_cur, 8, 0}; *width = 5; return 0;
-        case DOCKAUV_F_POOL_CAPSULES: *fd = {h->B.p_caps, c.max_capsules * 7, 0}; *width = c.max_capsules * 7; return 0;
-        case DOCKAUV_F_POOL_SPHERES: *fd = {h->B.p_sph, c.max_spheres * 4, 0}; *width = c.max_spheres * 4; return 0;
+        case DOCKAUV_F_STATE: *fd = {h->B.state, 12, 0, kVecPair}; *width = 12; return 0;
+        case DOCKAUV_F_U: *fd = {h->B.u, kMaxU, 0, kVecPair}; *width = kMaxU; return 0;
+        case DOCKAUV_F_GOAL: *fd = {h->B.goal, 4, 0, kVecPair}; *width = 4; return 0;
+        case DOCKAUV_F_CURRENT: *fd = {h->B.cur, 8, 0, kVecPair}; *width = 5; return 0;
+        case DOCKAUV_F_TSTEPS: *fd = {h->B.t_steps, 1, 1, 1}; *width = 1; return 0;
+        case DOCKAUV_F_CAPSULES: *fd = {h->B.caps, c.max_capsules * 7, 0, 1}; *width = c.max_capsules * 7; return 0;
+        case DOCKAUV_F_SPHERES: *fd = {h->B.sph, c.max_spheres * 4, 0, kVecQuad}; *width = c.max_spheres * 4; return 0;
+        case DOCKAUV_F_VEHICLE_ID: *fd = {h->B.veh_id, 1, 2, 1}; *width = 1; return 0;
+        case DOCKAUV_F_CUM_REWARD: *fd = {h->B.cum_reward, 1, 0, 1}; *width = 1; return 0;
+        case DOCKAUV_F_EPISODE: *fd = {h->B.episode, 1, 1, 1}; *width = 1; return 0;
+        case DOCKAUV_F_CURRENT_SIGMA: *fd = {h->B.cur_sigma, 1, 0, 1}; *width = 1; return 0;
+        case DOCKAUV_F_POOL_POSE: *fd = {h->B.p_pose, 6, 0, kVecPair}; *width = 6; return 0;
+        case DOCKAUV_F_POOL_GOAL: *fd = {h->B.p_goal, 4, 0, kVecPair}; *width = 4; return 0;
+        case DOCKAUV_F_POOL_CURRENT: *fd = {h->B.p_cur, 8, 0, kVecPair}; *width = 5; return 0;
+        case DOCKAUV_F_POOL_CAPSULES: *fd = {h->B.p_caps, c.max_capsules * 7, 0, 1}; *width = c.max_capsules * 7; return 0;
+        case DOCKAUV_F_POOL_SPHERES: *fd = {h->B.p_sph, c.max_spheres * 4, 0, kVecQuad}; *width = c.max_spheres * 4; return 0;
     }
     return fail(h, DOCKAUV_E_INVALID, "unknown field id %d", field);
 }
@@ -211,6 +212,20 @@
     if (kind == 0) return h->f64 ? static_cast<const double*>(src)[idx] : (double)static_cast<const float*>(src)[idx];
     if (kind == 1) return (double)static_cast<const int32_t*>(src)[idx];
     return (double)static_cast<const uint8_t*>(src)[idx];
+}
+
+int copy_rows(dockauv_handle h, void* base, int rows, int vec, size_t es, int first, int count, void* host, bool to_device) {
+    const size_t vrows = (size_t)(rows + vec - 1) / vec, run = (size_t)count * vec * es, pitch = (size_t)h->S * vec * es;
+    unsigned char* dev = static_cast<unsigned char*>(base) + vrow_index(vec, 0, (size_t)first, (size_t)h->S) * es;
+    if (to_device) HIP_TRY(h, hipMemcpy2D(dev, pitch, host, run, run, vrows, hipMemcpyHostToDevice));
+    else HIP_TRY(h, hipMemcpy2D(host, run, dev, pitch, run, vrows, hipMemcpyDeviceToHost));
+    return 0;
+}
+int zero_rows(dockauv_handle h, void* base, int rows, int vec, size_t es, int first, int count) {
+    const size_t vrows = (size_t)(rows + vec - 1) / vec, run = (size_t)count * vec * es, pitch = (size_t)h->S * vec * es;
+    unsigned char* dev = static_cast<unsigned char*>(base) + vrow_index(vec, 0, (size_t)first, (size_t)h->S) * es;
+    HIP_TRY(h, hipMemset2D(dev, pitch, 0, run, vrows));
+    return 0;
 }
 
 void set_io(StepIO& d, const dockauv_step_io& s) {
@@ -271,7 +286,8 @@
     if (c.envs_per_group == -1) h->sym = false;
 
     const size_t S = (size_t)h->S, t = h->tsz, N = (size_t)c.n_envs;
-    const size_t caps = (size_t)c.max_capsules * 7 * S * t, sph = (size_t)c.max_spheres * 4 * S * t;
+    const size_t caps = (size_t)c.max_capsules * 7 * S * t, sph = vrow_elems(kVecQuad, (size_t)c.max_spheres * 4, S) * t;
+    const auto pairs = [&](size_t rows) { return vrow_elems(kVecPair, rows, S) * t; };
     Buffers& B = h->B;
     B.stride = h->S;
     void *rays_dev = nullptr, *lt_dev = nullptr, *lc_dev = nullptr, *pdev = nullptr;
@@ -280,10 +296,10 @@
                                           N * h->n_rays * t, N * h->n_obs * 4, N * 12 * t};
     for (int k = 0; k < ST_COUNT; ++k) h->stage[k].bytes = stage_bytes[k];
     const struct { void** p; size_t bytes; } device_arrays[] = {
-        {&B.state, 12 * S * t}, {&B.pos_lo, kLoRows * S * t}, {&B.u, kMaxU * S * t}, {&B.goal, 4 * S * t}, {&B.cur, 8 * S * t},
+        {&B.state, pairs(12)}, {&B.pos_lo, pairs(kLoRows)}, {&B.u, pairs(kMaxU)}, {&B.goal, pairs(4)}, {&B.cur, pairs(8)},
         {&B.cum_reward, S * t}, {(void**)&B.t_steps, S * 4}, {(void**)&B.episode, S * 4}, {(void**)&B.veh_id, S},
-        {&B.cur_sigma, S * t}, {&B.caps, caps}, {&B.sph, sph}, {&B.p_pose, 6 * S * t}, {&B.p_goal, 4 * S * t},
-        {&B.p_cur, 8 * S * t}, {&B.p_caps, caps}, {&B.p_sph, sph}, {&rays_dev, (size_t)h->n_rays * 4 * t},
+        {&B.cur_sigma, S * t}, {&B.caps, caps}, {&B.sph, sph}, {&B.p_pose, pairs(6)}, {&B.p_goal, pairs(4)},
+        {&B.p_cur, pairs(8)}, {&B.p_caps, caps}, {&B.p_sph, sph}, {&rays_dev, (size_t)h->n_rays * 4 * t},
         {&lt_dev, (size_t)64 * 4 * t}, {&lc_dev, (size_t)64 * 4}, {&pdev, pbytes}};
     for (const auto& d : device_arrays)
         if (int rc = dalloc(h, d.p, d.bytes)) return rc;
@@ -498,29 +514,28 @@
     if (count == 0 || fd.rows == 0) return 0;
     HIP_TRY(h, hipSetDevice(h->device));
     const size_t es = elem_size(h, fd.kind);
-    std::vector<unsigned char> tmp((size_t)fd.rows * count * es);
+    const size_t n = (size_t)count;
+    std::vector<unsigned char> tmp(vrow_elems(fd.vec, fd.rows, n) * es);
     if (is_current_field(field)) {
         for (int i = 0; i < count; ++i) {
             const double* s = src + (size_t)i * 5;
             const double a = s[3], b = s[4];
             const double row[8] = {s[0], std::cos(a) * std::cos(b), std::sin(b), std::sin(a) * std::cos(b), s[1], s[2], a, b};
-            for (int k = 0; k < 8; ++k) store_elem(h, 0, tmp.data(), (size_t)k * count + i, row[k]);
+            for (int k = 0; k < 8; ++k) store_elem(h, 0, tmp.data(), vrow_index(fd.vec, k, i, n), row[k]);
         }
     } else {
         for (int i = 0; i < count; ++i)
-            for (int k = 0; k < width; ++k) store_elem(h, fd.kind, tmp.data(), (size_t)k * count + i, src[(size_t)i * width + k]);
-    }
-    unsigned char* dst = static_cast<unsigned char*>(fd.base) + (size_t)first * es;
-    HIP_TRY(h, hipMemcpy2D(dst, (size_t)h->S * es, tmp.data(), (size_t)count * es, (size_t)count * es, fd.rows, hipMemcpyHostToDevice));
+            for (int k = 0; k < width; ++k) store_elem(h, fd.kind, tmp.data(), vrow_index(fd.vec, k, i, n), src[(size_t)i * width + k]);
+    }
+    if ((rc = copy_rows(h, fd.base, fd.rows, fd.vec, es, first, count, tmp.data(), true)) != 0) return rc;
     if (field == DOCKAUV_F_STATE) {
-        std::vector<unsigned char> lo((size_t)kLoRows * count * es);
+        std::vector<unsigned char> lo(vrow_elems(kVecPair, kLoRows, n) * es);
         for (int i = 0; i < count; ++i)
             for (int k = 0; k < kLoRows; ++k) {
                 const double x = src[(size_t)i * width + kLoState[k]];
-                store_elem(h, 0, lo.data(), (size_t)k * count + i, h->f64 ? 0.0 : x - (double)(float)x);
+                store_elem(h, 0, lo.data(), vrow_index(kVecPair, k, i, n), h->f64 ? 0.0 : x - (double)(float)x);
             }
-        unsigned char* dlo = static_cast<unsigned char*>(h->B.pos_lo) + (size_t)first * es;
-        HIP_TRY(h, hipMemcpy2D(dlo, (size_t)h->S * es, lo.data(), (size_t)count * es, (size_t)count * es, kLoRows, hipMemcpyHostToDevice));
+        if ((rc = copy_rows(h, h->B.pos_lo, kLoRows, kVecPair, es, first, count, lo.data(), true)) != 0) return rc;
     }
     return 0;
 }
@@ -536,23 +551,22 @@
     HIP_TRY(h, hipSetDevice(h->device));
     if ((rc = sync_last(h)) != 0 || (rc = check_status(h)) != 0) return rc;
     const size_t es = elem_size(h, fd.kind);
-    std::vector<unsigned char> tmp((size_t)fd.rows * count * es);
-    const unsigned char* srcp = static_cast<const unsigned char*>(fd.base) + (size_t)first * es;
-    HIP_TRY(h, hipMemcpy2D(tmp.data(), (size_t)count * es, srcp, (size_t)h->S * es, (size_t)count * es, fd.rows, hipMemcpyDeviceToHost));
+    const size_t n = (size_t)count;
+    std::vector<unsigned char> tmp(vrow_elems(fd.vec, fd.rows, n) * es);
+    if ((rc = copy_rows(h, fd.base, fd.rows, fd.vec, es, first, count, tmp.data(), false)) != 0) return rc;
     if (is_current_field(field)) {
         static const int rows[5] = {0, 4, 5, 6, 7};
         for (int i = 0; i < count; ++i)
-            for (int k = 0; k < 5; ++k) dst[(size_t)i * 5 + k] = load_elem(h, 0, tmp.data(), (size_t)rows[k] * count + i);
+            for (int k = 0; k < 5; ++k) dst[(size_t)i * 5 + k] = load_elem(h, 0, tmp.data(), vrow_index(fd.vec, rows[k], i, n));
     } else {
         for (int i = 0; i < count; ++i)
-            for (int k = 0; k < width; ++k) dst[(size_t)i * width + k] = load_elem(h, fd.kind, tmp.data(), (size_t)k * count + i);
+            for (int k = 0; k < width; ++k) dst[(size_t)i * width + k] = load_elem(h, fd.kind, tmp.data(), vrow_index(fd.vec, k, i, n));
     }
     if (field == DOCKAUV_F_STATE && !h->f64) {
-        std::vector<unsigned char> lo((size_t)kLoRows * count * es);
-        const unsigned char* slo = static_cast<const unsigned char*>(h->B.pos_lo) + (size_t)first * es;
-        HIP_TRY(h, hipMemcpy2D(lo.data(), (size_t)count * es, slo, (size_t)h->S * es, (size_t)count * es, kLoRows, hipMemcpyDeviceToHost));
+        std::vector<unsigned char> lo(vrow_elems(kVecPair, kLoRows, n) * es);
+        if ((rc = copy_rows(h, h->B.pos_lo, kLoRows, kVecPair, es, first, count, lo.data(), false)) != 0) return rc;
         for (int i = 0; i < count; ++i)
-            for (int k = 0; k < kLoRows; ++k) dst[(size_t)i * width + kLoState[k]] += load_elem(h, 0, lo.data(), (size_t)k * count + i);
+            for (int k = 0; k < kLoRows; ++k) dst[(size_t)i * width + kLoState[k]] += load_elem(h, 0, lo.data(), vrow_index(kVecPair, k, i, n));
     }
     return 0;
 }
@@ -563,10 +577,10 @@
     if (count == 0) return 0;
     HIP_TRY(h, hipSetDevice(h->device));
     if (int rc = sync_last(h)) return rc;
-    const size_t t = h->tsz, S = (size_t)h->S;
-    HIP_TRY(h, hipMemset2D(static_cast<unsigned char*>(h->B.state) + first * t, S * t, 0, count * t, 12));
-    HIP_TRY(h, hipMemset2D(static_cast<unsigned char*>(h->B.pos_lo) + first * t, S * t, 0, count * t, kLoRows));
-    HIP_TRY(h, hipMemset2D(static_cast<unsigned char*>(h->B.u) + first * t, S * t, 0, count * t, kMaxU));
+    const size_t t = h->tsz;
+    if (int rc = zero_rows(h, h->B.state, 12, kVecPair, t, first, count)) return rc;
+    if (int rc = zero_rows(h, h->B.pos_lo, kLoRows, kVecPair, t, first, count)) return rc;
+    if (int rc = zero_rows(h, h->B.u, kMaxU, kVecPair, t, first, count)) return rc;
     HIP_TRY(h, hipMemset(static_cast<unsigned char*>(h->B.cum_reward) + first * t, 0, count * t));
     HIP_TRY(h, hipMemset(h->B.t_steps + first, 0, count * 4));
     std::vector<int32_t> ep(count);
diff --git a/gym_dockauv_amd/csrc/dockauv_device.h b/gym_dockauv_amd/csrc/dockauv_device.h
--- a/gym_dockauv_amd/csrc/dockauv_device.h
+++ b/gym_dockauv_amd/csrc/dockauv_device.h
@@ -53,6 +53,19 @@
     int device_noise;
     T fan_cos, fan_sin, sum_beta;
 };
+
+#if defined(__HIPCC__)
+#define DOCKAUV_HD __host__ __device__
+#else
+#define DOCKAUV_HD
+#endif
+
+constexpr int kVecPair = 2;
+constexpr int kVecQuad = 4;
+DOCKAUV_HD constexpr size_t vrow_index(int V, size_t k, size_t i, size_t S) { return ((k / V) * S + i) * V + k % V; }
+template <int V>
+DOCKAUV_HD constexpr size_t vrow_index(size_t k, size_t i, size_t S) { return vrow_index(V, k, i, S); }
+DOCKAUV_HD constexpr size_t vrow_elems(int V, size_t rows, size_t S) { return (rows + V - 1) / V * V * S; }
 
 struct Buffers {
     void* state;
diff --git a/gym_dockauv_amd/csrc/dockauv_step.hip.inc b/gym_dockauv_amd/csrc/dockauv_step.hip.inc
--- a/gym_dockauv_amd/csrc/dockauv_step.hip.inc
+++ b/gym_dockauv_amd/csrc/dockauv_step.hip.inc
@@ -126,6 +126,73 @@
         asm volatile("global_store_dwordx4 %0, %1, %2 sc1" ::"v"(byte_off), "v"(r), "s"(base) : "memory");
     else
         asm volatile("global_store_dwordx4 %0, %1, %2" ::"v"(byte_off), "v"(r), "s"(base) : "memory");
+}
+template <typename P, int V> using vec_ = P __attribute__((ext_vector_type(V)));
+template <int V, typename P>
+__device__ __forceinline__ P* vrow_base_(void* array, int env0, long S) { return static_cast<P*>(array) + vrow_index<V>(0, (size_t)env0, (size_t)S); }
+template <int V, typename P>
+__device__ __forceinline__ const P* vrow_base_(const void* array, int env0, long S) { return static_cast<const P*>(array) + vrow_index<V>(0, (size_t)env0, (size_t)S); }
+template <int V, typename P>
+__device__ __forceinline__ unsigned vrow_off_(int k, long S, unsigned lane) {
+    return (unsigned)vrow_index<V>((size_t)k, (size_t)lane, (size_t)(unsigned)S) * (unsigned)sizeof(P);
+}
+template <int AF, int V, typename P>
+__device__ __forceinline__ vec_<P, V> ldv_(const P* base, int r, long S, unsigned lane) {
+    typedef __attribute__((address_space(1))) const char* gcp;
+    return *reinterpret_cast<__attribute__((address_space(1))) const vec_<P, V>*>(
+        reinterpret_cast<gcp>(uniform_(reinterpret_cast<const char*>(base))) + vrow_off_<V, P>(r * V, S, lane));
+}
+template <int AF, int V, typename P>
+__device__ __forceinline__ void stv_(P* base, int r, long S, unsigned lane, vec_<P, V> v) {
+    typedef __attribute__((address_space(1))) char* gcp;
+    gcp p = reinterpret_cast<gcp>(uniform_(reinterpret_cast<char*>(base))) + vrow_off_<V, P>(r * V, S, lane);
+    if (DOCKAUV_WT_STORES && !(AF & kAfWriteBack)) {
+        typedef unsigned long long u64;
+        constexpr int N = (int)(V * sizeof(P) / 8);
+        static_assert(V * sizeof(P) % 8 == 0, "whole 8-byte pieces");
+        u64 w[N];
+        __builtin_memcpy(w, &v, sizeof(w));
+#pragma unroll
+        for (int j = 0; j < N; ++j)
+            __hip_atomic_store(reinterpret_cast<__attribute__((address_space(1))) u64*>(p) + j, w[j], __ATOMIC_RELAXED, __HIP_MEMORY_SCOPE_AGENT);
+    } else {
+        *reinterpret_cast<__attribute__((address_space(1))) vec_<P, V>*>(p) = v;
+    }
+}
+template <int AF, int V, typename P>
+__device__ __forceinline__ P lde_(const P* base, int k, long S, unsigned lane) {
+    typedef __attribute__((address_space(1))) const char* gcp;
+    return *reinterpret_cast<__attribute__((address_space(1))) const P*>(
+        reinterpret_cast<gcp>(uniform_(reinterpret_cast<const char*>(base))) + vrow_off_<V, P>(k, S, lane));
+}
+template <int AF, int V, typename P, typename X>
+__device__ __forceinline__ void ste_(P* base, int k, long S, unsigned lane, X v) {
+    typedef __attribute__((address_space(1))) char* gcp;
+    store_global_<AF>(reinterpret_cast<__attribute__((address_space(1))) P*>(
+        reinterpret_cast<gcp>(uniform_(reinterpret_cast<char*>(base))) + vrow_off_<V, P>(k, S, lane)), (P)v);
+}
+template <int AF, int NMAX, typename P>
+__device__ __forceinline__ void ld_pairs_(const P* base, int k0, int n, long S, unsigned lane, P* x) {
+#pragma unroll
+    for (int k = 0; k < NMAX; k += 2) {
+        if (k < n) {
+            const vec_<P, 2> v = ldv_<AF, 2>(base, (k0 + k) / 2, S, lane);
+            x[k] = v.x;
+            if (k + 1 < NMAX) x[k + 1] = (k + 1 < n) ? v.y : x[k + 1];
+        }
+    }
+}
+template <int AF, int NMAX, typename P>
+__device__ __forceinline__ void st_pairs_(P* base, int k0, int n, long S, unsigned lane, const P* x) {
+#pragma unroll
+    for (int k = 0; k < NMAX; k += 2) {
+        if (k + 1 < n) {
+            const vec_<P, 2> v = {x[k], x[k + 1 < NMAX ? k + 1 : k]};
+            stv_<AF, 2>(base, (k0 + k) / 2, S, lane, v);
+        } else if (k < n) {
+            ste_<AF, 2>(base, k0 + k, S, lane, x[k]);
+        }
+    }
 }
 template <typename P>
 __device__ __forceinline__ P ldg_(const P* base, long k, long S, unsigned lane) { return ldgx_<0>(base, k, S, lane); }
@@ -375,7 +442,7 @@
 template <typename T, int VK, bool SYM, int VOFF, bool HOTV = false, typename VP, typename EP, typename REQ = NoFetch, typename PIN = NoFetch,
           typename REQT = NoFetch>
 __device__ __forceinline__ void vehicle_step_(const VP& V, const EP& E, T y[9], T dpos[3], T u[kMaxU],
-                                              const T act[kMaxU], const T nuc[3], T* g_u, long S, unsigned ul, T& psi_lo,
+                                              const T act[kMaxU], const T nuc[3], T* v_u, long S, unsigned ul, T& psi_lo,
                                               const REQ& request_kinetics = REQ(), const PIN& pin_kinetics = PIN(),
                                               const REQT& request_tail = REQT()) {
     const int n_u = (VK == VK_LAUV) ? 3 : (VK == VK_JOY ? 6 : V.n_u);
@@ -386,14 +453,15 @@
             const T a = clip_(act[i], T(-1), T(1));
             const T x = V.ulo[i] + V.uhalf[i] * ((a + T(1)) * T(0.5));
             u[i] = E.lp_alpha * x + one_m_alpha * u[i];
-            if (!HOTV) stgx_<VOFF>(g_u, i, S, ul, u[i]);
-        }
-    }
-    if (HOTV) {
-#pragma unroll
-        for (int i = 0; i < kMaxU; ++i)
-            if (i < n_u) stgx_<VOFF>(g_u, i, S, ul, u[i]);
-    }
+            if (!HOTV) {
+                if ((i & 1) || i == n_u - 1) {
+                    const vec_<T, 2> up = {u[i & ~1], u[(i & ~1) + 1]};
+                    stv_<VOFF, kVecPair>(v_u, i / 2, S, ul, up);
+                }
+            }
+        }
+    }
+    if (HOTV) st_pairs_<VOFF, kMaxU>(v_u, 0, (n_u + 1) & ~1, S, ul, u);
     T tau_c[6] = {0, 0, 0, 0, 0, 0};
     if (VK == VK_JOY) {
 #pragma unroll
@@ -972,14 +1040,14 @@
     T oa_den_r = T(0);
 
     const unsigned ul = (unsigned)(tid % EPG);
-    T* g_state = static_cast<T*>(B.state) + env0;
-    T* g_plo = static_cast<T*>(B.pos_lo) + env0;
-    T* g_u = static_cast<T*>(B.u) + env0;
-    T* g_goal = static_cast<T*>(B.goal) + env0;
-    T* g_cur = static_cast<T*>(B.cur) + env0;
+    T* v_state = vrow_base_<kVecPair, T>(B.state, env0, S);
+    T* v_plo = vrow_base_<kVecPair, T>(B.pos_lo, env0, S);
+    T* v_u = vrow_base_<kVecPair, T>(B.u, env0, S);
+    T* v_goal = vrow_base_<kVecPair, T>(B.goal, env0, S);
+    T* v_cur = vrow_base_<kVecPair, T>(B.cur, env0, S);
     T* g_cum = static_cast<T*>(B.cum_reward) + env0;
     T* g_caps = static_cast<T*>(B.caps) + env0;
-    T* g_sph = static_cast<T*>(B.sph) + env0;
+    T* v_sph = vrow_base_<kVecQuad, T>(B.sph, env0, S);
     int32_t* g_tsteps = B.t_steps + env0;
     int32_t* g_episode = B.episode + env0;
     constexpr int NU_CT = (VK == VK_LAUV) ? 3 : ((VK == VK_DENSEB) ? 0 : 6);
@@ -1051,31 +1119,33 @@
     if (RAISE_PRIO && wv == 0) __builtin_amdgcn_s_setprio(kPrioLevel);
     if (loader) {
         if (VK == VK_MIXED) vid_l = ldgx_<VOFF>(B.veh_id + env0, 0, S, ul);
-#pragma unroll
-        for (int k = 0; k < 12; ++k)
-            if (!(LATE_GOAL && k < 3)) st[k] = ldgx_<VOFF>(g_state, k, S, ul);
-        if (sizeof(T) == 4 && !LATE_GOAL) {
-#pragma unroll
-            for (int k = 0; k < 3; ++k) plo[k] = ldgx_<VOFF>(g_plo, k, S, ul);
-        }
-        if (sizeof(T) == 4) psi_lo = ldgx_<VOFF>(g_plo, 3, S, ul);
+        if (LATE_GOAL) {
+            st[3] = lde_<VOFF, kVecPair>(v_state, 3, S, ul);
+            ld_pairs_<VOFF, 8>(v_state, 4, 8, S, ul, st + 4);
+        } else {
+            ld_pairs_<VOFF, 12>(v_state, 0, 12, S, ul, st);
+        }
+        if (sizeof(T) == 4) {
+            if (LATE_GOAL) {
+                psi_lo = lde_<VOFF, kVecPair>(v_plo, 3, S, ul);
+            } else {
+                const vec_<T, 2> l0 = ldv_<VOFF, kVecPair>(v_plo, 0, S, ul), l1 = ldv_<VOFF, kVecPair>(v_plo, 1, S, ul);
+                plo[0] = l0.x; plo[1] = l0.y; plo[2] = l1.x; psi_lo = l1.y;
+            }
+        }
         const T* actp = static_cast<const T*>(IO.actions) + (size_t)env0 * n_u_max;
 #pragma unroll
-        for (int k = 0; k < kMaxU; ++k) {
-            if (k < n_u_max) {
-                u[k] = ldgx_<VOFF>(g_u, k, S, ul);
-                act[k] = actp[ul * (unsigned)n_u_max + k];
-            } else {
-                u[k] = T(0);
-                act[k] = T(0);
-            }
-        }
-        Vc = ldgx_<VOFF>(g_cur, 0, S, ul);
-        cdx = ldgx_<VOFF>(g_cur, 1, S, ul); cdy = ldgx_<VOFF>(g_cur, 2, S, ul); cdz = ldgx_<VOFF>(g_cur, 3, S, ul);
-        vmin = ldgx_<VOFF>(g_cur, 4, S, ul); vmax = ldgx_<VOFF>(g_cur, 5, S, ul);
+        for (int k = 0; k < kMaxU; ++k) u[k] = T(0);
+        ld_pairs_<VOFF, kMaxU>(v_u, 0, (n_u_max + 1) & ~1, S, ul, u);
+#pragma unroll
+        for (int k = 0; k < kMaxU; ++k) act[k] = k < n_u_max ? actp[ul * (unsigned)n_u_max + k] : T(0);
+        {
+            const vec_<T, 2> c0 = ldv_<VOFF, kVecPair>(v_cur, 0, S, ul), c1 = ldv_<VOFF, kVecPair>(v_cur, 1, S, ul),
+                             c2 = ldv_<VOFF, kVecPair>(v_cur, 2, S, ul);
+            Vc = c0.x; cdx = c0.y; cdy = c1.x; cdz = c1.y; vmin = c2.x; vmax = c2.y;
+        }
         if (!LATE_GOAL) {
-#pragma unroll
-            for (int k = 0; k < 4; ++k) goal[k] = ldgx_<VOFF>(g_goal, k, S, ul);
+            ld_pairs_<VOFF, 4>(v_goal, 0, 4, S, ul, goal);
             t_steps = ldgx_<VOFF>(g_tsteps, 0, S, ul);
         }
         w_noise = IO.noise ? ldgx_<VOFF>(static_cast<const T*>(IO.noise) + env0, 0, S, ul) : T(0);
@@ -1111,16 +1181,14 @@
     }
     if (bk_lane || rs_lane) {
         if (!SHARE_NAV) {
-#pragma unroll
-            for (int k = 0; k < 4; ++k) goal_b[k] = ldgx_<VOFF>(g_goal, k, S, ule);
+            ld_pairs_<VOFF, 4>(v_goal, 0, 4, S, ule, goal_b);
         }
         t_steps_b = ldgx_<VOFF>(g_tsteps, 0, S, ule);
         cum_in = ldgx_<VOFF>(g_cum, 0, S, ule);
         episode_in = ldgx_<VOFF>(g_episode, 0, S, ule);
     }
     if (QUAD && ob_lane && !SHARE_NAV) {
-#pragma unroll
-        for (int k = 0; k < 4; ++k) goal_o[k] = ldgx_<VOFF>(g_goal, k, S, ule);
+        ld_pairs_<VOFF, 4>(v_goal, 0, 4, S, ule, goal_o);
         t_steps_o = ldgx_<VOFF>(g_tsteps, 0, S, ule);
     }
 
@@ -1183,12 +1251,12 @@
             int nsph = 0;
             bool open = true;
             for (int s_i = 0; s_i < E.max_sph; ++s_i) {
-                T rad = T(0);
-#pragma unroll
-                for (int k = 0; k < 4; ++k) {
-                    rad = ldgx_<VOFF>(g_sph, s_i * 4 + k, S, (unsigned)pe);
-                    lds_sph[(size_t)(s_i * kSphFields + k) * EPG + pe] = rad;
-                }
+                const vec_<T, 4> sp = ldv_<VOFF, kVecQuad>(v_sph, s_i, S, (unsigned)pe);
+                const T rad = sp.w;
+                lds_sph[(size_t)(s_i * kSphFields + 0) * EPG + pe] = sp.x;
+                lds_sph[(size_t)(s_i * kSphFields + 1) * EPG + pe] = sp.y;
+                lds_sph[(size_t)(s_i * kSphFields + 2) * EPG + pe] = sp.z;
+                lds_sph[(size_t)(s_i * kSphFields + 3) * EPG + pe] = rad;
                 open = open && (rad > T(0));
                 nsph = open ? s_i + 1 : nsph;
             }
@@ -1247,18 +1315,18 @@
             }
         }
         if constexpr (HOT) {
-            vehicle_step_<T, VK, SYM, VOFF, true>(HR.V, HR, st + 3, dpos, u, act, nuc, g_u, S, ul, psi_lo,
+            vehicle_step_<T, VK, SYM, VOFF, true>(HR.V, HR, st + 3, dpos, u, act, nuc, v_u, S, ul, psi_lo,
                                                   [&]() { request_hot_kinetics_<T, VK>(PB->H[0], HR); },
                                                   [&]() { pin_hot_kinetics_<T, VK>(HR); },
                                                   [&]() { if constexpr (TAIL) request_tail_<G0>(PB->Q, Q, RC, RQ); });
         } else if (VK == VK_MIXED) {
             if (vid == 0) {
-                vehicle_step_<T, VK_JOY, SYM, VOFF>(PB->V[0], E, st + 3, dpos, u, act, nuc, g_u, S, ul, psi_lo);
+                vehicle_step_<T, VK_JOY, SYM, VOFF>(PB->V[0], E, st + 3, dpos, u, act, nuc, v_u, S, ul, psi_lo);
             } else {
-                vehicle_step_<T, VK_LAUV, SYM, VOFF>(PB->V[1], E, st + 3, dpos, u, act, nuc, g_u, S, ul, psi_lo);
+                vehicle_step_<T, VK_LAUV, SYM, VOFF>(PB->V[1], E, st + 3, dpos, u, act, nuc, v_u, S, ul, psi_lo);
             }
         } else {
-            vehicle_step_<T, VK, SYM, VOFF>(PB->V[0], E, st + 3, dpos, u, act, nuc, g_u, S, ul, psi_lo);
+            vehicle_step_<T, VK, SYM, VOFF>(PB->V[0], E, st + 3, dpos, u, act, nuc, v_u, S, ul, psi_lo);
         }
         auto update_position = [&]() {
 #pragma unroll
@@ -1277,14 +1345,9 @@
         if (!LATE_GOAL) update_position();
         DOCKAUV_STAMP_PIN(3, st + 3, 9);
         if (LATE_GOAL) {
-#pragma unroll
-            for (int k = 0; k < 3; ++k) st[k] = ldgx_<VOFF>(g_state, k, S, ul);
-            if (sizeof(T) == 4) {
-#pragma unroll
-                for (int k = 0; k < 3; ++k) plo[k] = ldgx_<VOFF>(g_plo, k, S, ul);
-            }
-#pragma unroll
-            for (int k = 0; k < 4; ++k) goal[k] = ldgx_<VOFF>(g_goal, k, S, ul);
+            ld_pairs_<VOFF, 3>(v_state, 0, 3, S, ul, st);
+            if (sizeof(T) == 4) ld_pairs_<VOFF, 3>(v_plo, 0, 3, S, ul, plo);
+            ld_pairs_<VOFF, 4>(v_goal, 0, 4, S, ul, goal);
             t_steps = ldgx_<VOFF>(g_tsteps, 0, S, ul);
         }
         g1 = RAYS ? trig_accurate_(st[3], st[4], st[5]) : trig_(st[3], st[4], st[5]);
@@ -1563,14 +1626,13 @@
             if (RAYS) obs_ray_cells(zero_row, ul);
         }
         if (DUAL && !zero_row) {
-#pragma unroll
-            for (int k = 0; k < 12; ++k) stgx_<VOFF>(g_state, k, S, ul, st[k]);
-            stgx_<VOFF>(g_cur, 0, S, ul, Vc);
+            st_pairs_<VOFF, 12>(v_state, 0, 12, S, ul, st);
+            const vec_<T, 2> c0 = {Vc, cdx};
+            stv_<VOFF, kVecPair>(v_cur, 0, S, ul, c0);
         }
         if (sizeof(T) == 4) {
-#pragma unroll
-            for (int k = 0; k < 3; ++k) stgx_<VOFF>(g_plo, k, S, ul, zero_row ? T(0) : plo[k]);
-            stgx_<VOFF>(g_plo, 3, S, ul, zero_row ? T(0) : psi_lo);
+            const T lo[4] = {zero_row ? T(0) : plo[0], zero_row ? T(0) : plo[1], zero_row ? T(0) : plo[2], zero_row ? T(0) : psi_lo};
+            st_pairs_<VOFF, 4>(v_plo, 0, 4, S, ul, lo);
         }
         DOCKAUV_STAMP(5);
     };
@@ -1746,19 +1808,16 @@
             const int ep_next = episode_in + 1;
             T curv[8];
             if (LOG && Q.reset_mode == 1) {
-                const T* pp = static_cast<const T*>(B.p_pose);
-                const T* pg = static_cast<const T*>(B.p_goal);
-                const T* pc = static_cast<const T*>(B.p_cur);
-#pragma unroll
-                for (int k = 0; k < 6; ++k) sb[k] = ldgx_<VOFF>(pp + env0, k, S, ule);
-#pragma unroll
-                for (int k = 0; k < 4; ++k) goal_b[k] = ldgx_<VOFF>(pg + env0, k, S, ule);
-#pragma unroll
-                for (int k = 0; k < 8; ++k) curv[k] = ldgx_<VOFF>(pc + env0, k, S, ule);
+                const T* pp = vrow_base_<kVecPair, T>(B.p_pose, env0, S);
+                const T* pg = vrow_base_<kVecPair, T>(B.p_goal, env0, S);
+                const T* pc = vrow_base_<kVecPair, T>(B.p_cur, env0, S);
+                ld_pairs_<VOFF, 6>(pp, 0, 6, S, ule, sb);
+                ld_pairs_<VOFF, 4>(pg, 0, 4, S, ule, goal_b);
+                ld_pairs_<VOFF, 8>(pc, 0, 8, S, ule, curv);
                 const T* pcap = static_cast<const T*>(B.p_caps);
                 for (int k = 0; k < E.max_cap * 7; ++k) stgx_<VOFF>(g_caps, (size_t)k, S, ule, ldgx_<VOFF>(pcap + env0, (size_t)k, S, ule));
-                const T* psp = static_cast<const T*>(B.p_sph);
-                for (int k = 0; k < E.max_sph * 4; ++k) stgx_<VOFF>(g_sph, (size_t)k, S, ule, ldgx_<VOFF>(psp + env0, (size_t)k, S, ule));
+                const T* psp = vrow_base_<kVecQuad, T>(B.p_sph, env0, S);
+                for (int s_i = 0; s_i < E.max_sph; ++s_i) stv_<VOFF, kVecQuad>(v_sph, s_i, S, ule, ldv_<VOFF, kVecQuad>(psp, s_i, S, ule));
             } else {
                 T ring_s;
                 if (DUAL) {
@@ -1778,20 +1837,19 @@
             }
 #pragma unroll
             for (int k = 6; k < 12; ++k) sb[k] = T(0);
-#pragma unroll
-            for (int k = 0; k < kMaxU; ++k)
-                if (k < n_u_max) stgx_<VOFF>(g_u, k, S, ule, T(0));
-#pragma unroll
-            for (int k = 0; k < 4; ++k) stgx_<VOFF>(g_goal, k, S, ule, goal_b[k]);
-#pragma unroll
-            for (int k = 1; k < 8; ++k) stgx_<VOFF>(g_cur, k, S, ule, curv[k]);
+            const T uz[kMaxU] = {};
+            st_pairs_<VOFF, kMaxU>(v_u, 0, (n_u_max + 1) & ~1, S, ule, uz);
+            st_pairs_<VOFF, 4>(v_goal, 0, 4, S, ule, goal_b);
+            st_pairs_<VOFF, 8>(v_cur, 0, 8, S, ule, curv);
             Vc_b = curv[0];
             stgx_<VOFF>(g_episode, 0, S, ule, ep_next);
         }
         if (!DUAL || reset_now) {
-#pragma unroll
-            for (int k = 0; k < 12; ++k) stgx_<VOFF>(g_state, k, S, ule, sb[k]);
-            stgx_<VOFF>(g_cur, 0, S, ule, Vc_b);
+            st_pairs_<VOFF, 12>(v_state, 0, 12, S, ule, sb);
+            if (!reset_now) {
+                const vec_<T, 2> c0 = {Vc_b, cdx};
+                stv_<VOFF, kVecPair>(v_cur, 0, S, ule, c0);
+            }
         }
     };
 
```

Result: no change. 7.568 billion (-0.4%).
